# facebookresearch/detectron2

Hardware: NVIDIA H100
Metric: Mask R-CNN R50-FPN training hot-path images/sec (custom-op path fwd+bwd, 2 images/GPU) (higher is better)
Workload: dtype f32

## Files before the change

detectron2_b200/_C.py:

```python
import ctypes as C
import os

import torch

_HERE = os.path.dirname(os.path.abspath(__file__))
LIB_PATH = os.path.join(_HERE, "libd2b200.so")

_lib = None

D2B_ERRORS = {-1: "invalid argument", -2: "workspace too small", -3: "unsupported configuration"}


class DcnParams(C.Structure):
    _fields_ = [(n, C.c_int) for n in ("N", "Cin", "H", "W", "Cout", "kh", "kw", "stride_h", "stride_w", "pad_h",
                                        "pad_w", "dil_h", "dil_w", "groups", "deformable_groups")]


MAX_LEVELS = 8
MAX_IMAGES = 64
ABI_VERSION = 4
DCN_X_NHWC = 1
ROI_ROTATED, ROI_BACKWARD = 1, 2
DTYPE_CODE = {torch.float32: 0, torch.float16: 1, torch.bfloat16: 2}
MATCH_ROTATED, MATCH_LOW_QUALITY, MATCH_APPEND_GT = 1, 2, 4
MATCH_MAX_THRESHOLDS = 8


class Pyramid(C.Structure):
    _fields_ = [("num_levels", C.c_int), ("feat", C.c_void_p * MAX_LEVELS), ("grad", C.c_void_p * MAX_LEVELS),
                ("H", C.c_int * MAX_LEVELS), ("W", C.c_int * MAX_LEVELS), ("scale", C.c_float * MAX_LEVELS),
                ("min_level", C.c_int), ("max_level", C.c_int), ("canonical_level", C.c_int),
                ("canonical_box_size", C.c_float), ("level_rois", C.c_void_p)]


class RpnLevels(C.Structure):
    _fields_ = [("num_levels", C.c_int), ("proposals", C.c_void_p * MAX_LEVELS), ("topk_idx", C.c_void_p * MAX_LEVELS),
                ("topk_scores", C.c_void_p * MAX_LEVELS), ("A", C.c_int * MAX_LEVELS), ("k", C.c_int * MAX_LEVELS)]


class DenseLevels(C.Structure):
    _fields_ = [("num_levels", C.c_int), ("anchors", C.c_void_p * MAX_LEVELS), ("deltas", C.c_void_p * MAX_LEVELS),
                ("topk_idx", C.c_void_p * MAX_LEVELS), ("topk_scores", C.c_void_p * MAX_LEVELS),
                ("R", C.c_int * MAX_LEVELS), ("k", C.c_int * MAX_LEVELS)]


LABELS_I8, LABELS_I64 = 0, 1
SAMPLE_MAX_SAMPLES = 8192
LOSS_STATUS_INVALID_BOX, LOSS_STATUS_INVALID_CLASS, LOSS_STATUS_INVALID_BOX_ORDER = 1, 2, 4
LOSS_TYPES = {"smooth_l1": 0, "giou": 1}


class DenseLossLevels(C.Structure):
    _fields_ = [("num_levels", C.c_int), ("logits", C.c_void_p * MAX_LEVELS), ("deltas", C.c_void_p * MAX_LEVELS),
                ("grad_logits", C.c_void_p * MAX_LEVELS), ("grad_deltas", C.c_void_p * MAX_LEVELS),
                ("R", C.c_int * MAX_LEVELS)]


def _declare(lib):
    vp, f32p, i64p, u8p = C.c_void_p, C.c_void_p, C.c_void_p, C.c_void_p
    i, f, d, sz, i64 = C.c_int, C.c_float, C.c_double, C.c_size_t, C.c_int64
    sig = {
        "d2b_abi_version": (i, []),
        "d2b_cuda_version": (i, []),
        "d2b_arch": (C.c_char_p, []),
        "d2b_roi_align_forward": (i, [f32p, i, i, i, i, f32p, i, f, i, i, i, i, f32p, vp]),
        "d2b_roi_align_backward": (i, [f32p, f32p, i, f, i, i, i, i, i, i, i, i, f32p, vp]),
        "d2b_roi_pooler_forward": (i, [C.POINTER(Pyramid), i, i, f32p, i, i, i, i, i, f32p, vp]),
        "d2b_roi_pooler_backward": (i, [C.POINTER(Pyramid), i, i, f32p, f32p, i, i, i, i, i, vp]),
        "d2b_roi_align_forward_nhwc": (i, [f32p, i, i, i, i, f32p, i, f, i, i, i, i, f32p, vp]),
        "d2b_roi_pooler_forward_nhwc": (i, [C.POINTER(Pyramid), i, i, f32p, i, i, i, i, i, f32p, vp]),
        "d2b_pyramid_nchw_to_nhwc": (i, [C.POINTER(Pyramid), i, i, C.POINTER(C.c_void_p), vp]),
        "d2b_pyramid_nhwc_to_nchw": (i, [C.POINTER(Pyramid), i, i, C.POINTER(C.c_void_p), vp]),
        "d2b_pyramid_nchw_to_nhwc_t": (i, [C.POINTER(Pyramid), i, i, C.POINTER(C.c_void_p), i, vp]),
        "d2b_pyramid_nhwc_to_nchw_t": (i, [C.POINTER(Pyramid), i, i, C.POINTER(C.c_void_p), i, vp]),
        "d2b_roi_pooler_forward_nhwc_t": (i, [C.POINTER(Pyramid), i, i, f32p, i, i, i, i, i, vp, i, vp]),
        "d2b_roi_pooler_backward_nhwc_t": (i, [C.POINTER(Pyramid), i, i, vp, i, f32p, i, i, i, i, i, vp]),
        "d2b_roi_align_backward_nhwc": (i, [f32p, f32p, i, f, i, i, i, i, i, i, i, i, f32p, vp]),
        "d2b_roi_pooler_backward_nhwc": (i, [C.POINTER(Pyramid), i, i, f32p, f32p, i, i, i, i, i, vp]),
        "d2b_roi_align_rotated_forward": (i, [f32p, i, i, i, i, f32p, i, f, i, i, i, f32p, vp]),
        "d2b_roi_align_rotated_backward": (i, [f32p, f32p, i, f, i, i, i, i, i, i, i, f32p, vp]),
        "d2b_roi_align_rotated_forward_nhwc": (i, [f32p, i, i, i, i, f32p, i, f, i, i, i, f32p, vp]),
        "d2b_roi_align_rotated_backward_nhwc": (i, [f32p, f32p, i, f, i, i, i, i, i, i, i, f32p, vp]),
        "d2b_roi_pooler_rotated_forward": (i, [C.POINTER(Pyramid), i, i, f32p, i, i, i, i, f32p, vp]),
        "d2b_roi_pooler_rotated_backward": (i, [C.POINTER(Pyramid), i, i, f32p, f32p, i, i, i, i, vp]),
        "d2b_roi_pooler_rotated_forward_nhwc_t": (i, [C.POINTER(Pyramid), i, i, f32p, i, i, i, i, vp, i, vp]),
        "d2b_roi_pooler_rotated_backward_nhwc_t": (i, [C.POINTER(Pyramid), i, i, vp, i, f32p, i, i, i, i, vp]),
        "d2b_roi_pooler_nhwc_supported": (i, [C.POINTER(Pyramid), i, i, i, i]),
        "d2b_nms_workspace_bytes": (sz, [i64, i, i64]),
        "d2b_nms": (i, [f32p, f32p, i64p, i64, d, i, i64, i64p, i64p, vp, sz, vp]),
        "d2b_rpn_prepare": (i, [C.POINTER(RpnLevels), i, f32p, f, i, f32p, f32p, f32p, f32p, i64p, vp, vp]),
        "d2b_rpn_select": (i, [i64p, i64p, i, i, i, f32p, f32p, i64p, f32p, f32p, i64p, i64p, vp]),
        "d2b_frcnn_prepare": (i, [f32p, f32p, C.POINTER(C.c_int), i, i, i, f32p, f, i, f32p, f32p, f32p, f32p, i64p, i64p,
                                  i64p, i64p, vp]),
        "d2b_dense_prepare": (i, [C.POINTER(DenseLevels), i, i, C.POINTER(C.c_float), f, f32p, f32p, f32p, f32p, i64p, i64p,
                                  vp]),
        "d2b_rrpn_prepare": (i, [C.POINTER(RpnLevels), i, f32p, f, i, f32p, f32p, f32p, f32p, i64p, vp, vp]),
        "d2b_frcnn_rotated_prepare": (i, [f32p, f32p, C.POINTER(C.c_int), i, i, i, f32p, f, i, i, f32p, f32p, f32p, f32p, i64p,
                                          i64p, i64p, i64p, vp]),
        "d2b_rpn_select_rotated": (i, [i64p, i64p, i, i, i, f32p, f32p, i64p, f32p, f32p, i64p, i64p, vp]),
        "d2b_mask_loss_forward": (i, [f32p, i, i, i, u8p, i, i, i, f32p, i64p, i64p, f32p, u8p, vp]),
        "d2b_mask_loss_backward": (i, [f32p, i, i, i, u8p, i64p, f32p, f32p, vp]),
        "d2b_keypoints_workspace_bytes": (sz, [i, i]),
        "d2b_keypoints_from_heatmaps": (i, [f32p, i, i, i, f32p, f32p, vp, sz, vp]),
        "d2b_keypoint_loss_forward": (i, [vp, i, i, i, i, f32p, f32p, i64p, u8p, f32p, i64p, vp]),
        "d2b_keypoint_loss_backward": (i, [vp, i, i, i, i, i64p, u8p, f32p, vp, vp]),
        "d2b_dense_loss_workspace_bytes": (sz, [C.POINTER(DenseLossLevels), i, i, i]),
        "d2b_dense_loss_forward": (i, [C.POINTER(DenseLossLevels), i, i, i, i, f32p, f32p, vp, i, f, f, f, i, f,
                                       C.POINTER(C.c_float), f32p, f32p, i64p, i64p, vp, vp, sz, vp]),
        "d2b_dense_loss_backward": (i, [C.POINTER(DenseLossLevels), i, i, i, i, f32p, f32p, vp, i, f, f, f, i, f,
                                        C.POINTER(C.c_float), f32p, f32p, vp]),
        "d2b_frcnn_loss_workspace_bytes": (sz, [i]),
        "d2b_frcnn_loss_forward": (i, [vp, vp, i, i, i, i, i, f32p, f32p, i64p, f, i, f, C.POINTER(C.c_float), f32p, f32p, i64p,
                                       i64p, i64p, i64p, vp, vp, sz, vp]),
        "d2b_frcnn_loss_backward": (i, [vp, vp, i, i, i, i, i, f32p, f32p, i64p, f, i, f, C.POINTER(C.c_float), f32p, f32p, vp,
                                        vp, vp]),
        "d2b_box_iou_rotated": (i, [f32p, i64, f32p, i64, f32p, vp]),
        "d2b_match_workspace_bytes": (sz, [i, i, i]),
        "d2b_match_boxes": (i, [f32p, i64p, i, i, f32p, i64, i64p, i, C.POINTER(C.c_double), i, C.POINTER(C.c_int), i, f32p, d,
                                i64p, i64, i64p, vp, f32p, i64p, vp, vp, sz, vp]),
        "d2b_sample_labels_workspace_bytes": (sz, [i, i, i]),
        "d2b_sample_labels": (i, [vp, i, i, i, i64, i, i, vp, vp, i64p, i64p, i64p, vp, sz, vp]),
        "d2b_deform_conv_tc_shape_supported": (i, [C.POINTER(DcnParams), i]),
        "d2b_deform_conv_forward_workspace_bytes": (sz, [C.POINTER(DcnParams), i, i]),
        "d2b_deform_conv_cols_bytes": (sz, [C.POINTER(DcnParams), i]),
        "d2b_deform_conv_forward": (i, [f32p, f32p, f32p, f32p, f32p, C.POINTER(DcnParams), i, i, f32p, vp, vp, sz, vp]),
        "d2b_deform_conv_backward_workspace_bytes": (sz, [C.POINTER(DcnParams), i, i, i, i]),
        "d2b_deform_conv_backward": (i, [f32p, f32p, f32p, f32p, f32p, C.POINTER(DcnParams), i, i, vp, f32p, f32p, f32p,
                                         f32p, f32p, vp, sz, vp]),
        "d2b_deform_conv_fused_forward": (i, [f32p, f32p, f32p, f32p, f32p, i, C.POINTER(DcnParams), i, i, f32p, vp, vp, sz,
                                              vp]),
        "d2b_deform_conv_fused_backward": (i, [f32p, f32p, f32p, f32p, i, f32p, f32p, C.POINTER(DcnParams), i, i, vp, f32p,
                                               f32p, f32p, vp, sz, vp]),
        "d2b_paste_masks": (i, [f32p, f32p, i, i, i, i, f, u8p, vp]),
        "d2b_paste_masks_packed": (i, [f32p, f32p, i, i, i, i, f, vp, vp]),
    }
    for name, (res, args) in sig.items():
        fn = getattr(lib, name)
        fn.restype = res
        fn.argtypes = args
    return sig


EXPORTED = None


def lib():
    global _lib, EXPORTED
    if _lib is None:
        if not os.path.exists(LIB_PATH):
            raise RuntimeError(
                "detectron2_b200: native library %s is missing. Build it with `python -m detectron2_b200.build` "
                "(or __graft_entry__.build()). There is no CPU / PyTorch fallback for these ops." % LIB_PATH)
        l = C.CDLL(LIB_PATH)
        EXPORTED = _declare(l)
        if l.d2b_abi_version() != ABI_VERSION:
            raise RuntimeError("libd2b200.so ABI version mismatch")
        _lib = l
    return _lib


def check(rc, what):
    if rc == 0:
        return
    if rc < 0:
        raise RuntimeError("%s: %s (d2b error %d)" % (what, D2B_ERRORS.get(rc, "error"), rc))
    raise RuntimeError("%s: CUDA error %d" % (what, rc))


def stream_ptr(device):
    return C.c_void_p(torch.cuda.current_stream(device).cuda_stream)


def ptr(t):
    return None if t is None else C.c_void_p(t.data_ptr())


def require_cuda(*tensors):
    for t in tensors:
        if t is not None and not t.is_cuda:
            raise NotImplementedError("detectron2_b200 ops run on CUDA tensors only (no CPU fallback)")


def get_cuda_version():
    v = lib().d2b_cuda_version()
    return "CUDA %d.%d" % (v // 1000, (v % 1000) // 10)


def has_cuda():
    return True


def get_compiler_version():
    return "nvcc (sm_90a)"


DCN_PRECISION = -1


def _into(dst, src):
    if dst.shape != src.shape:
        dst.resize_(src.shape)
    dst.copy_(src)


def deform_conv_forward(input, weight, offset, output, columns, ones, kW, kH, dW, dH, padW, padH, dilW, dilH, group,
                        deformable_group, im2col_step):
    from . import ops

    if weight.shape[3] != kW or weight.shape[2] != kH:
        raise RuntimeError("deform_conv_forward: kernel size does not match the weight tensor")
    y = ops.deform_conv_op(input, offset, None, weight, None, [dH, dW], [padH, padW], [dilH, dilW], group, deformable_group,
                           DCN_PRECISION)
    _into(output, y)
    return 1


def deform_conv_backward_input(input, offset, gradOutput, gradInput, gradOffset, weight, columns, kW, kH, dW, dH, padW,
                               padH, dilW, dilH, group, deformable_group, im2col_step):
    from . import ops

    gx, go, _, _, _ = ops.deform_conv_backward_op(input, offset, None, weight, gradOutput, [dH, dW], [padH, padW],
                                                  [dilH, dilW], group, deformable_group, False, True, False, DCN_PRECISION)
    _into(gradInput, gx)
    _into(gradOffset, go)
    return 1


def deform_conv_backward_filter(input, offset, gradOutput, gradWeight, columns, ones, kW, kH, dW, dH, padW, padH, dilW,
                                dilH, group, deformable_group, scale, im2col_step):
    from . import ops

    _, _, _, gw, _ = ops.deform_conv_backward_op(input, offset, None, gradWeight.new_empty(gradWeight.shape), gradOutput,
                                                 [dH, dW], [padH, padW], [dilH, dilW], group, deformable_group, False,
                                                 False, True, DCN_PRECISION)
    gradWeight.add_(gw, alpha=float(scale))
    return 1


def modulated_deform_conv_forward(input, weight, bias, ones, offset, mask, output, columns, kernel_h, kernel_w, stride_h,
                                  stride_w, pad_h, pad_w, dilation_h, dilation_w, group, deformable_group, with_bias):
    from . import ops

    y = ops.deform_conv_op(input, offset, mask, weight, bias if with_bias else None, [stride_h, stride_w], [pad_h, pad_w],
                           [dilation_h, dilation_w], group, deformable_group, DCN_PRECISION)
    _into(output, y)


def modulated_deform_conv_backward(input, weight, bias, ones, offset, mask, columns, grad_input, grad_weight, grad_bias,
                                   grad_offset, grad_mask, grad_output, kernel_h, kernel_w, stride_h, stride_w, pad_h,
                                   pad_w, dilation_h, dilation_w, group, deformable_group, with_bias):
    from . import ops

    gx, go, gm, gw, gb = ops.deform_conv_backward_op(input, offset, mask, weight, grad_output, [stride_h, stride_w],
                                                     [pad_h, pad_w], [dilation_h, dilation_w], group, deformable_group,
                                                     bool(with_bias), True, True, DCN_PRECISION)
    _into(grad_input, gx)
    _into(grad_offset, go)
    _into(grad_mask, gm)
    grad_weight.add_(gw)
    if with_bias:
        grad_bias.add_(gb)
```

detectron2_b200/csrc/deform_conv.cu:

```cuda
#include "common.cuh"
#include "deform_conv_tc.cuh"

namespace {

constexpr int BN = 64;
constexpr int BM = 64;
constexpr int BK = 16;
constexpr int kThreads = 256;

struct Dims {
  int N, Cin, H, W, Cout, kh, kw, sh, sw, ph, pw, dh, dw, G, DG, Ho, Wo;
  int cpg, opg, cpdg, KK, HoWo;
};

inline bool make_dims(const d2b_dcn_params* p, Dims& d) {
  if (!p) return false;
  d.N = p->N; d.Cin = p->Cin; d.H = p->H; d.W = p->W; d.Cout = p->Cout; d.kh = p->kh; d.kw = p->kw;
  d.sh = p->stride_h; d.sw = p->stride_w; d.ph = p->pad_h; d.pw = p->pad_w; d.dh = p->dil_h; d.dw = p->dil_w;
  d.G = p->groups; d.DG = p->deformable_groups;
  if (d.N < 0 || d.Cin <= 0 || d.H <= 0 || d.W <= 0 || d.Cout <= 0 || d.kh <= 0 || d.kw <= 0 || d.sh <= 0 ||
      d.sw <= 0 || d.ph < 0 || d.pw < 0 || d.dh <= 0 || d.dw <= 0 || d.G <= 0 || d.DG <= 0)
    return false;
  if (d.Cin % d.G || d.Cout % d.G || d.Cin % d.DG) return false;
  d.Ho = (d.H + 2 * d.ph - (d.dh * (d.kh - 1) + 1)) / d.sh + 1;
  d.Wo = (d.W + 2 * d.pw - (d.dw * (d.kw - 1) + 1)) / d.sw + 1;
  if (d.Ho <= 0 || d.Wo <= 0) return false;
  d.cpg = d.Cin / d.G; d.opg = d.Cout / d.G; d.cpdg = d.Cin / d.DG; d.KK = d.kh * d.kw; d.HoWo = d.Ho * d.Wo;
  return true;
}

struct TapTile {
  int pos[4][BN];
  float wgt[4][BN];
  float msk[BN];
  float fh[BN], fw[BN];
  int inside[BN];
};

__device__ __forceinline__ void build_taps(TapTile& t, const Dims& d, const float* __restrict__ offset,
                                           const float* __restrict__ mask, int b, int dg, int kp, int p0) {
  for (int n = threadIdx.x; n < BN; n += kThreads) {
    const int p = p0 + n;
    int pos[4] = {-1, -1, -1, -1};
    float w[4] = {0.f, 0.f, 0.f, 0.f};
    float m = 1.f, lh = 0.f, lw = 0.f;
    int inside = 0;
    if (p < d.HoWo) {
      const int ho = p / d.Wo, wo = p - ho * d.Wo;
      const int i = kp / d.kw, j = kp - i * d.kw;
      const size_t obase = ((size_t)(b * d.DG + dg) * 2 * d.KK) * d.HoWo;
      const float oh = offset[obase + (size_t)(2 * kp) * d.HoWo + p];
      const float ow = offset[obase + (size_t)(2 * kp + 1) * d.HoWo + p];
      const float h = (float)(ho * d.sh - d.ph + i * d.dh) + oh;
      const float wv = (float)(wo * d.sw - d.pw + j * d.dw) + ow;
      if (mask) m = mask[((size_t)(b * d.DG + dg) * d.KK + kp) * d.HoWo + p];
      if (h > -1.f && wv > -1.f && h < (float)d.H && wv < (float)d.W) {
        inside = 1;
        const int hl = (int)floorf(h), wl = (int)floorf(wv);
        lh = h - (float)hl;
        lw = wv - (float)wl;
        const float hh = 1.f - lh, hw = 1.f - lw;
        const bool t0 = hl >= 0, t1 = hl + 1 <= d.H - 1, l0 = wl >= 0, l1 = wl + 1 <= d.W - 1;
        if (t0 && l0) { pos[0] = hl * d.W + wl; w[0] = hh * hw; }
        if (t0 && l1) { pos[1] = hl * d.W + wl + 1; w[1] = hh * lw; }
        if (t1 && l0) { pos[2] = (hl + 1) * d.W + wl; w[2] = lh * hw; }
        if (t1 && l1) { pos[3] = (hl + 1) * d.W + wl + 1; w[3] = lh * lw; }
      }
    }
#pragma unroll
    for (int q = 0; q < 4; ++q) {
      t.pos[q][n] = pos[q];
      t.wgt[q][n] = w[q];
    }
    t.msk[n] = m;
    t.fh[n] = lh;
    t.fw[n] = lw;
    t.inside[n] = inside;
  }
}

__device__ __forceinline__ float gather_val(const TapTile& t, const float* __restrict__ plane, int n) {
  float v = 0.f;
#pragma unroll
  for (int q = 0; q < 4; ++q) {
    const int pos = t.pos[q][n];
    if (pos >= 0) v += t.wgt[q][n] * __ldg(plane + pos);
  }
  return v;
}

__global__ void __launch_bounds__(kThreads) dcn_fwd_kernel(const float* __restrict__ x,
                                                           const float* __restrict__ offset,
                                                           const float* __restrict__ mask,
                                                           const float* __restrict__ weight,
                                                           const float* __restrict__ bias, Dims d,
                                                           float* __restrict__ out) {
  __shared__ TapTile taps;
  __shared__ float As[BK][BM + 4];
  __shared__ float Bs[BK][BN + 4];
  const int p0 = blockIdx.x * BN, m0 = blockIdx.y * BM;
  const int b = blockIdx.z / d.G, g = blockIdx.z - b * d.G;
  const int tid = threadIdx.x, tx = tid & 15, ty = tid >> 4;
  const int K = d.cpg * d.KK;
  float acc[4][4] = {};
  const int cbeg = g * d.cpg, cend = cbeg + d.cpg;
  for (int dg = cbeg / d.cpdg; dg * d.cpdg < cend; ++dg) {
    const int sbeg = max(cbeg, dg * d.cpdg), send = min(cend, (dg + 1) * d.cpdg);
    for (int kp = 0; kp < d.KK; ++kp) {
      __syncthreads();
      build_taps(taps, d, offset, mask, b, dg, kp, p0);
      __syncthreads();
      for (int c0 = sbeg; c0 < send; c0 += BK) {
        for (int e = tid; e < BK * BM; e += kThreads) {
          const int kk = e / BM, m = e - kk * BM;
          const int c = c0 + kk;
          float v = 0.f;
          if (c < send && m0 + m < d.opg) v = __ldg(weight + (size_t)(g * d.opg + m0 + m) * K + (c - cbeg) * d.KK + kp);
          As[kk][m] = v;
        }
        for (int e = tid; e < BK * BN; e += kThreads) {
          const int kk = e / BN, n = e - kk * BN;
          const int c = c0 + kk;
          float v = 0.f;
          if (c < send) v = gather_val(taps, x + ((size_t)b * d.Cin + c) * d.H * d.W, n) * taps.msk[n];
          Bs[kk][n] = v;
        }
        __syncthreads();
#pragma unroll
        for (int kk = 0; kk < BK; ++kk) {
          float a[4], bb[4];
#pragma unroll
          for (int i = 0; i < 4; ++i) a[i] = As[kk][ty * 4 + i];
#pragma unroll
          for (int j = 0; j < 4; ++j) bb[j] = Bs[kk][tx * 4 + j];
#pragma unroll
          for (int i = 0; i < 4; ++i)
#pragma unroll
            for (int j = 0; j < 4; ++j) acc[i][j] = fmaf(a[i], bb[j], acc[i][j]);
        }
        __syncthreads();
      }
    }
  }
#pragma unroll
  for (int i = 0; i < 4; ++i) {
    const int m = m0 + ty * 4 + i;
    if (m >= d.opg) continue;
    const int oc = g * d.opg + m;
    const float bv = bias ? bias[oc] : 0.f;
#pragma unroll
    for (int j = 0; j < 4; ++j) {
      const int p = p0 + tx * 4 + j;
      if (p < d.HoWo) out[((size_t)b * d.Cout + oc) * d.HoWo + p] = acc[i][j] + bv;
    }
  }
}

__global__ void __launch_bounds__(kThreads) dcn_bwd_data_kernel(const float* __restrict__ x,
                                                                const float* __restrict__ offset,
                                                                const float* __restrict__ mask,
                                                                const float* __restrict__ weight,
                                                                const float* __restrict__ gout, Dims d,
                                                                float* __restrict__ gx, float* __restrict__ goff,
                                                                float* __restrict__ gmask) {
  __shared__ TapTile taps;
  __shared__ float Ws[BK][BK + 1];
  __shared__ float Gs[BK][BN + 4];
  __shared__ float red[3][4][BN];
  const int p0 = blockIdx.x * BN;
  const int b = blockIdx.z / d.G, g = blockIdx.z - b * d.G;
  const int tid = threadIdx.x, n = tid & 63, kq = tid >> 6;
  const int K = d.cpg * d.KK;
  const int cbeg = g * d.cpg, cend = cbeg + d.cpg;
  const size_t plane = (size_t)d.H * d.W;
  for (int dg = cbeg / d.cpdg; dg * d.cpdg < cend; ++dg) {
    const int sbeg = max(cbeg, dg * d.cpdg), send = min(cend, (dg + 1) * d.cpdg);
    for (int kp = 0; kp < d.KK; ++kp) {
      __syncthreads();
      build_taps(taps, d, offset, mask, b, dg, kp, p0);
      __syncthreads();
      float s_h = 0.f, s_w = 0.f, s_m = 0.f;
      for (int c0 = sbeg + (int)blockIdx.y * BK; c0 < send; c0 += BK * (int)gridDim.y) {
        float acc[4] = {0.f, 0.f, 0.f, 0.f};
        for (int mm0 = 0; mm0 < d.opg; mm0 += BK) {
          {
            const int m = tid >> 4, kk = tid & 15;
            const int c = c0 + kk;
            float v = 0.f;
            if (c < send && mm0 + m < d.opg)
              v = __ldg(weight + (size_t)(g * d.opg + mm0 + m) * K + (c - cbeg) * d.KK + kp);
            Ws[m][kk] = v;
          }
          for (int e = tid; e < BK * BN; e += kThreads) {
            const int m = e / BN, nn = e - m * BN;
            float v = 0.f;
            if (mm0 + m < d.opg && p0 + nn < d.HoWo)
              v = __ldg(gout + ((size_t)b * d.Cout + g * d.opg + mm0 + m) * d.HoWo + p0 + nn);
            Gs[m][nn] = v;
          }
          __syncthreads();
#pragma unroll
          for (int m = 0; m < BK; ++m) {
            const float gv = Gs[m][n];
#pragma unroll
            for (int i = 0; i < 4; ++i) acc[i] = fmaf(Ws[m][kq + 4 * i], gv, acc[i]);
          }
          __syncthreads();
        }
        if (taps.inside[n]) {
          const float mk = taps.msk[n], lh = taps.fh[n], lw = taps.fw[n];
          const int q0 = taps.pos[0][n], q1 = taps.pos[1][n], q2 = taps.pos[2][n], q3 = taps.pos[3][n];
#pragma unroll
          for (int i = 0; i < 4; ++i) {
            const int c = c0 + kq + 4 * i;
            if (c >= send) continue;
            const float gc = acc[i];
            const float gm = gc * mk;
            const float* __restrict__ xp = x + ((size_t)b * d.Cin + c) * plane;
            float* __restrict__ gp = gx ? gx + ((size_t)b * d.Cin + c) * plane : nullptr;
            const float v0 = q0 >= 0 ? __ldg(xp + q0) : 0.f, v1 = q1 >= 0 ? __ldg(xp + q1) : 0.f;
            const float v2 = q2 >= 0 ? __ldg(xp + q2) : 0.f, v3 = q3 >= 0 ? __ldg(xp + q3) : 0.f;
            if (gp) {
              if (q0 >= 0) atomicAdd(gp + q0, gm * taps.wgt[0][n]);
              if (q1 >= 0) atomicAdd(gp + q1, gm * taps.wgt[1][n]);
              if (q2 >= 0) atomicAdd(gp + q2, gm * taps.wgt[2][n]);
              if (q3 >= 0) atomicAdd(gp + q3, gm * taps.wgt[3][n]);
            }
            s_h += gm * ((1.f - lw) * (v2 - v0) + lw * (v3 - v1));
            s_w += gm * ((1.f - lh) * (v1 - v0) + lh * (v3 - v2));
            s_m += gc * (taps.wgt[0][n] * v0 + taps.wgt[1][n] * v1 + taps.wgt[2][n] * v2 + taps.wgt[3][n] * v3);
          }
        }
      }
      red[0][kq][n] = s_h;
      red[1][kq][n] = s_w;
      red[2][kq][n] = s_m;
      __syncthreads();
      if (tid < 3 * BN) {
        const int which = tid / BN, nn = tid - which * BN;
        const int p = p0 + nn;
        if (p < d.HoWo) {
          const float v = red[which][0][nn] + red[which][1][nn] + red[which][2][nn] + red[which][3][nn];
          if (which < 2) {
            if (goff) atomicAdd(goff + ((size_t)(b * d.DG + dg) * 2 * d.KK + 2 * kp + which) * d.HoWo + p, v);
          } else if (gmask && mask) {
            atomicAdd(gmask + ((size_t)(b * d.DG + dg) * d.KK + kp) * d.HoWo + p, v);
          }
        }
      }
    }
  }
}

__global__ void __launch_bounds__(kThreads) dcn_bwd_weight_kernel(const float* __restrict__ x,
                                                                  const float* __restrict__ offset,
                                                                  const float* __restrict__ mask,
                                                                  const float* __restrict__ gout, Dims d,
                                                                  int tiles_per_cta, int n_ctile,
                                                                  float* __restrict__ gw) {
  __shared__ TapTile taps;
  __shared__ float Gs[BN][BM + 4];
  __shared__ float Cs[BN][BK + 1];
  const int g = blockIdx.z;
  const int mt = blockIdx.y / n_ctile, ct = blockIdx.y - mt * n_ctile;
  const int m0 = mt * BM;
  const int cbeg = g * d.cpg;
  const int c0 = cbeg + ct * BK;
  const int cend = min(cbeg + d.cpg, c0 + BK);
  const int tid = threadIdx.x, tm = tid >> 2, tc = tid & 3;
  const int K = d.cpg * d.KK;
  const int ptiles = d2b_cdiv(d.HoWo, BN);
  const int total_tiles = d.N * ptiles;
  const int t_begin = blockIdx.x * tiles_per_cta, t_end = min(total_tiles, t_begin + tiles_per_cta);
  for (int kp = 0; kp < d.KK; ++kp) {
    float acc[4] = {0.f, 0.f, 0.f, 0.f};
    for (int t = t_begin; t < t_end; ++t) {
      const int b = t / ptiles, p0 = (t - b * ptiles) * BN;
      for (int cs = c0; cs < cend;) {
        const int dg = cs / d.cpdg;
        const int ce = min(cend, (dg + 1) * d.cpdg);
        __syncthreads();
        build_taps(taps, d, offset, mask, b, dg, kp, p0);
        for (int e = tid; e < BN * BM; e += kThreads) {
          const int nn = e & 63, m = e >> 6;
          float v = 0.f;
          if (m0 + m < d.opg && p0 + nn < d.HoWo)
            v = __ldg(gout + ((size_t)b * d.Cout + g * d.opg + m0 + m) * d.HoWo + p0 + nn);
          Gs[nn][m] = v;
        }
        __syncthreads();
        for (int e = tid; e < BN * BK; e += kThreads) {
          const int nn = e & 63, kk = e >> 6;
          const int c = c0 + kk;
          float v = 0.f;
          if (c >= cs && c < ce) v = gather_val(taps, x + ((size_t)b * d.Cin + c) * d.H * d.W, nn) * taps.msk[nn];
          Cs[nn][kk] = v;
        }
        __syncthreads();
#pragma unroll 8
        for (int nn = 0; nn < BN; ++nn) {
          const float gv = Gs[nn][tm];
#pragma unroll
          for (int i = 0; i < 4; ++i) acc[i] = fmaf(gv, Cs[nn][tc * 4 + i], acc[i]);
        }
        cs = ce;
      }
    }
    if (m0 + tm < d.opg) {
#pragma unroll
      for (int i = 0; i < 4; ++i) {
        const int c = c0 + tc * 4 + i;
        if (c < cend) atomicAdd(gw + (size_t)(g * d.opg + m0 + tm) * K + (c - cbeg) * d.KK + kp, acc[i]);
      }
    }
  }
}

__global__ void __launch_bounds__(256) dcn_bias_grad_kernel(const float* __restrict__ gout, int N, int Cout, int HoWo,
                                                            float* __restrict__ gb) {
  __shared__ float s[8];
  const int oc = blockIdx.x;
  float v = 0.f;
  for (int b = 0; b < N; ++b)
    for (int p = threadIdx.x; p < HoWo; p += 256) v += gout[((size_t)b * Cout + oc) * HoWo + p];
  for (int o = 16; o; o >>= 1) v += __shfl_xor_sync(0xffffffffu, v, o);
  if ((threadIdx.x & 31) == 0) s[threadIdx.x >> 5] = v;
  __syncthreads();
  if (threadIdx.x == 0) {
    float t = 0.f;
    for (int i = 0; i < 8; ++i) t += s[i];
    gb[oc] = t;
  }
}

}

D2B_API int d2b_deform_conv_tc_shape_supported(const d2b_dcn_params* p, int backward) {
  return backward ? d2b_deform_conv_tc_bwd_supported(p) : d2b_deform_conv_tc_supported(p);
}

D2B_API size_t d2b_deform_conv_forward_workspace_bytes(const d2b_dcn_params* p, int precision, int flags) {
  if (precision == 0) return 0;
  if (precision == -1 && !d2b_deform_conv_tc_supported(p)) return 0;
  return d2b_deform_conv_tc_fwd_workspace(p, (flags & D2B_DCN_X_NHWC) ? 1 : 0);
}

D2B_API size_t d2b_deform_conv_cols_bytes(const d2b_dcn_params* p, int precision) {
  if (precision == -1) precision = (d2b_deform_conv_tc_supported(p) && d2b_deform_conv_tc_bwd_supported(p)) ? 1 : 0;
  if (precision == 0 || !d2b_deform_conv_tc_bwd_supported(p)) return 0;
  return d2b_deform_conv_tc_cols_bytes(p, precision);
}

D2B_API int d2b_deform_conv_forward(const float* x, const float* offset, const float* mask, const float* weight,
                                    const float* bias, const d2b_dcn_params* p, int precision, int flags, float* out,
                                    void* cols, void* workspace, size_t workspace_bytes, void* stream) {
  Dims d;
  if (!make_dims(p, d)) return D2B_EINVAL;
  if (d.N == 0) return D2B_OK;
  if (!x || !offset || !weight || !out) return D2B_EINVAL;
  if (precision < -1 || precision > 2) return D2B_EINVAL;
  if (precision == -1) precision = d2b_deform_conv_tc_supported(p) ? 1 : 0;
  if (precision != 0)
    return d2b_deform_conv_forward_tc(x, offset, mask, weight, nullptr, bias, 0, p, precision,
                                      (flags & D2B_DCN_X_NHWC) ? 1 : 0, out, cols, workspace, workspace_bytes, stream);
  if (flags & D2B_DCN_X_NHWC) return D2B_EUNSUPPORTED;
  if (cols) return D2B_EINVAL;
  dim3 grid(d2b_cdiv(d.HoWo, BN), d2b_cdiv(d.opg, BM), d.N * d.G);
  dcn_fwd_kernel<<<grid, kThreads, 0, (cudaStream_t)stream>>>(x, offset, mask, weight, bias, d, out);
  D2B_CHECK_LAUNCH();
  return D2B_OK;
}

D2B_API size_t d2b_deform_conv_backward_workspace_bytes(const d2b_dcn_params* p, int precision, int flags, int need_data,
                                                        int need_weight) {
  if (precision == 0) return 0;
  if (precision == -1 && !d2b_deform_conv_tc_bwd_supported(p)) return 0;
  return d2b_deform_conv_tc_bwd_workspace(p, (flags & D2B_DCN_X_NHWC) ? 1 : 0, need_data, need_weight);
}

D2B_API int d2b_deform_conv_backward(const float* x, const float* offset, const float* mask, const float* weight,
                                     const float* grad_out, const d2b_dcn_params* p, int precision, int flags,
                                     const void* cols, float* grad_x, float* grad_offset, float* grad_mask,
                                     float* grad_weight, float* grad_bias, void* workspace, size_t workspace_bytes,
                                     void* stream_) {
  cudaStream_t stream = (cudaStream_t)stream_;
  Dims d;
  if (!make_dims(p, d)) return D2B_EINVAL;
  if (precision < -1 || precision > 2) return D2B_EINVAL;
  if (precision == -1) precision = d2b_deform_conv_tc_bwd_supported(p) ? 1 : 0;
  if (d.N > 0 && (!x || !offset || !weight || !grad_out)) return D2B_EINVAL;
  if (cols && precision == 0) return D2B_EINVAL;
  if (grad_bias) {
    if (d.N == 0) {
      D2B_CUDA(cudaMemsetAsync(grad_bias, 0, (size_t)d.Cout * 4, stream));
    } else {
      dcn_bias_grad_kernel<<<d.Cout, 256, 0, stream>>>(grad_out, d.N, d.Cout, d.HoWo, grad_bias);
      D2B_CHECK_LAUNCH();
    }
  }
  if (precision != 0)
    return d2b_deform_conv_backward_tc(x, offset, mask, weight, grad_out, nullptr, nullptr, 0, p, precision,
                                       (flags & D2B_DCN_X_NHWC) ? 1 : 0, cols, grad_x, grad_offset, grad_mask, grad_weight,
                                       workspace, workspace_bytes, stream_);
  if (flags & D2B_DCN_X_NHWC) return D2B_EUNSUPPORTED;
  const size_t nx = (size_t)d.N * d.Cin * d.H * d.W, noff = (size_t)d.N * d.DG * 2 * d.KK * d.HoWo;
  const size_t nm = (size_t)d.N * d.DG * d.KK * d.HoWo, nw = (size_t)d.Cout * d.cpg * d.KK;
  if (grad_x && nx) D2B_CUDA(cudaMemsetAsync(grad_x, 0, nx * 4, stream));
  if (grad_offset && noff) D2B_CUDA(cudaMemsetAsync(grad_offset, 0, noff * 4, stream));
  if (grad_mask && nm) D2B_CUDA(cudaMemsetAsync(grad_mask, 0, nm * 4, stream));
  if (grad_weight) D2B_CUDA(cudaMemsetAsync(grad_weight, 0, nw * 4, stream));
  if (d.N == 0) return D2B_OK;
  if (grad_x || grad_offset || grad_mask) {
    const int base_ctas = d2b_cdiv(d.HoWo, BN) * d.N * d.G;
    int csplit = d2b_cdiv(3LL * d2b_num_sms(), base_ctas);
    const int nchunks = d2b_cdiv(d.cpg, BK);
    if (csplit > nchunks) csplit = nchunks;
    if (csplit < 1) csplit = 1;
    dim3 grid(d2b_cdiv(d.HoWo, BN), csplit, d.N * d.G);
    dcn_bwd_data_kernel<<<grid, kThreads, 0, stream>>>(x, offset, mask, weight, grad_out, d, grad_x, grad_offset,
                                                       grad_mask);
    D2B_CHECK_LAUNCH();
  }
  if (grad_weight) {
    const int ptiles = d2b_cdiv(d.HoWo, BN), total = d.N * ptiles;
    const int n_ctile = d2b_cdiv(d.cpg, BK), n_mtile = d2b_cdiv(d.opg, BM);
    int per_tile_ctas = n_ctile * n_mtile * d.G;
    int splits = d2b_cdiv(4LL * d2b_num_sms(), per_tile_ctas);
    if (splits > total) splits = total;
    if (splits < 1) splits = 1;
    const int tiles_per_cta = d2b_cdiv(total, splits);
    splits = d2b_cdiv(total, tiles_per_cta);
    dim3 grid(splits, n_mtile * n_ctile, d.G);
    dcn_bwd_weight_kernel<<<grid, kThreads, 0, stream>>>(x, offset, mask, grad_out, d, tiles_per_cta, n_ctile,
                                                         grad_weight);
    D2B_CHECK_LAUNCH();
  }
  return D2B_OK;
}

D2B_API int d2b_deform_conv_fused_forward(const float* x, const float* offset_mask, const float* weight, const float* scale,
                                          const float* shift, int relu, const d2b_dcn_params* p, int precision, int flags,
                                          float* out, void* cols, void* workspace, size_t workspace_bytes, void* stream) {
  Dims d;
  if (!make_dims(p, d)) return D2B_EINVAL;
  if (d.N == 0) return D2B_OK;
  if (!x || !offset_mask || !weight || !out || precision == 0 || precision < -1 || precision > 2) return D2B_EINVAL;
  if (precision == -1) precision = 1;
  return d2b_deform_conv_forward_tc(x, offset_mask, nullptr, weight, scale, shift, relu, p, precision,
                                    ((flags & D2B_DCN_X_NHWC) ? 1 : 0) | 2, out, cols, workspace, workspace_bytes, stream);
}

D2B_API int d2b_deform_conv_fused_backward(const float* x, const float* offset_mask, const float* weight, const float* scale,
                                           int relu, const float* y, const float* grad_out, const d2b_dcn_params* p,
                                           int precision, int flags, const void* cols, float* grad_x,
                                           float* grad_offset_mask, float* grad_weight, void* workspace,
                                           size_t workspace_bytes, void* stream) {
  Dims d;
  if (!make_dims(p, d)) return D2B_EINVAL;
  if (precision == 0 || precision < -1 || precision > 2) return D2B_EINVAL;
  if (precision == -1) precision = 1;
  if (d.N > 0 && (!x || !offset_mask || !weight || !grad_out)) return D2B_EINVAL;
  return d2b_deform_conv_backward_tc(x, offset_mask, nullptr, weight, grad_out, scale, y, relu, p, precision,
                                     ((flags & D2B_DCN_X_NHWC) ? 1 : 0) | 2, cols, grad_x, grad_offset_mask, nullptr,
                                     grad_weight, workspace, workspace_bytes, stream);
}
```

detectron2_b200/csrc/deform_conv_tc.cu:

```cuda
#include <algorithm>
#include <cstdlib>

#include "common.cuh"
#include "deform_conv_tc.cuh"
#include "tc_common.cuh"

using namespace d2b_tc;

namespace {

constexpr int kWorkerWarps = 16;
constexpr int kWorkers = kWorkerWarps * 32;
constexpr int kThreads = kWorkers + 128;
constexpr int kLaunchRegs = (65536 / kThreads) & ~7;
constexpr int kWorkerRegs = 112, kSideRegs = 24;
static_assert(kWorkers * kWorkerRegs + (kThreads - kWorkers) * kSideRegs <= kThreads * kLaunchRegs,
              "register budget exceeds the launch allocation");
constexpr int kMaxBN = 128;
constexpr int kRowsPerHalf = 128 / (2 * kWorkerWarps);
constexpr int kTile = 16384;
constexpr int kMaxSmem = 227 * 1024;
constexpr int kGcolPitch = 132;

struct TC {
  int N, Cin, H, W, Cout, kh, kw, sh, sw, ph, pw, dh, dw, G, DG, Ho, Wo, cpg, opg, cpdg, KK, HoWo;
  int pack, SG, cps, ops, cbs, U;
  int tiles_img;
  int stages_img;
  int MC;
  int nks;
  long long off_bs, mask_bs;
  int mask_sigmoid;
};

struct Epi {
  const float* scale;
  const float* shift;
  int relu;
};

struct K1P { int BN, noct, goct, nkp, ksplit, S, tap_bytes, stage_bytes, red; };
struct K2P { int mper, msplit, tap_bytes; };
struct K3P { int BN, noct, sper, nsplit, S, stage_bytes; };

inline size_t align256(size_t v) { return (v + 255) & ~(size_t)255; }

bool make_tc(const d2b_dcn_params* p, TC& d) {
  if (!p) return false;
  d.N = p->N; d.Cin = p->Cin; d.H = p->H; d.W = p->W; d.Cout = p->Cout; d.kh = p->kh; d.kw = p->kw;
  d.sh = p->stride_h; d.sw = p->stride_w; d.ph = p->pad_h; d.pw = p->pad_w; d.dh = p->dil_h; d.dw = p->dil_w;
  d.G = p->groups; d.DG = p->deformable_groups;
  if (d.N < 0 || d.Cin <= 0 || d.H <= 0 || d.W <= 0 || d.Cout <= 0 || d.kh <= 0 || d.kw <= 0 || d.sh <= 0 || d.sw <= 0 ||
      d.ph < 0 || d.pw < 0 || d.dh <= 0 || d.dw <= 0 || d.G <= 0 || d.DG <= 0)
    return false;
  if (d.Cin % d.G || d.Cout % d.G || d.Cin % d.DG) return false;
  d.Ho = (d.H + 2 * d.ph - (d.dh * (d.kh - 1) + 1)) / d.sh + 1;
  d.Wo = (d.W + 2 * d.pw - (d.dw * (d.kw - 1) + 1)) / d.sw + 1;
  if (d.Ho <= 0 || d.Wo <= 0) return false;
  d.cpg = d.Cin / d.G; d.opg = d.Cout / d.G; d.cpdg = d.Cin / d.DG; d.KK = d.kh * d.kw; d.HoWo = d.Ho * d.Wo;
  if (d.cpg >= 64) {
    if (d.cpg % 64) return false;
    d.pack = 1;
  } else {
    if (d.cpg != 16 && d.cpg != 32) return false;
    d.pack = 64 / d.cpg;
    if (d.G % d.pack) return false;
  }
  if (d.cpdg % 64) return false;
  d.SG = d.G / d.pack; d.cps = d.cpg * d.pack; d.ops = d.opg * d.pack; d.cbs = d.cps / 64; d.U = d.KK * d.cbs;
  if (d.ops % 16) return false;
  if (d.KK > 49) return false;
  if ((long long)d.H * d.W * d.Cin >= (1LL << 29)) return false;
  if ((long long)d.HoWo * d.Cout >= (1LL << 31) || (long long)d.Cout * d.cpg * d.KK >= (1LL << 31)) return false;
  d.tiles_img = d2b_cdiv(d.HoWo, 128);
  d.stages_img = d2b_cdiv(d.HoWo, 64);
  d.MC = (d.U + 1) / 2;
  d.nks = d.ops / 64;
  if ((long long)d.N * d.tiles_img > 0x7fffffffLL) return false;
  d.off_bs = (long long)d.DG * 2 * d.KK * d.HoWo;
  d.mask_bs = (long long)d.DG * d.KK * d.HoWo;
  d.mask_sigmoid = 0;
  return true;
}

const float* use_fused_offset_mask(TC& d, const float* offset_mask) {
  d.off_bs = d.mask_bs = (long long)d.DG * 3 * d.KK * d.HoWo;
  d.mask_sigmoid = 1;
  return offset_mask + (size_t)d.DG * 2 * d.KK * d.HoWo;
}

int largest_tile(int n) {
  for (int t = kMaxBN; t >= 16; t >>= 1)
    if (n % t == 0) return t;
  return 0;
}

int best_split(long long base, int work, int max_split, int overhead) {
  int best = 1;
  long long best_cost = -1;
  for (int s = 1; s <= max_split; ++s) {
    const int per = d2b_cdiv(work, s);
    const int parts = d2b_cdiv(work, per);
    const long long cost = (long long)d2b_cdiv(base * parts, d2b_num_sms()) * (per + overhead);
    if (best_cost < 0 || cost < best_cost) {
      best_cost = cost;
      best = parts;
    }
  }
  return best;
}

bool plan_k1(const TC& d, K1P& k, bool colfed = false) {
  k.BN = largest_tile(d.ops);
  if (k.BN < 16) return false;
  k.noct = d.ops / k.BN;
  k.goct = colfed ? 1 : k.noct;
  const int base = d.N * d.tiles_img * d.SG * k.goct;
  k.ksplit = best_split(base, d.KK, d.KK, 1);
  k.nkp = d2b_cdiv(d.KK, k.ksplit);
  k.ksplit = d2b_cdiv(d.KK, k.nkp);
  k.red = k.ksplit > 1;
  const int ndg = d.DG == 1 ? 1 : std::min(d.DG, d2b_cdiv(d.cps, d.cpdg) + 1);
  k.tap_bytes = ndg * k.nkp * 128 * 16;
  k.stage_bytes = 2 * kTile + 2 * k.BN * 128;
  k.S = 3;
  while (k.S > 1 && k.S * k.stage_bytes + k.tap_bytes + 1024 + 128 > kMaxSmem) --k.S;
  return k.S >= 2;
}

bool plan_k1c(const TC& d, K1P& k1, K1P& kc) {
  const long long base = (long long)d.N * d.tiles_img * d.SG * (k1.noct - 1);
  if (k1.goct != 1 || k1.noct < 2 || (long long)d.N * d.tiles_img * (k1.noct - 1) > 0x7fffffffLL) return false;
  kc = k1;
  kc.goct = k1.noct - 1;
  kc.ksplit = best_split(base, d.KK, d.KK, 1);
  kc.nkp = d2b_cdiv(d.KK, kc.ksplit);
  kc.ksplit = d2b_cdiv(d.KK, kc.nkp);
  kc.tap_bytes = 0;
  kc.S = 3;
  while (kc.S > 1 && kc.S * kc.stage_bytes + 1024 + 128 > kMaxSmem) --kc.S;
  if (kc.S < 2) return false;
  k1.red = kc.red = k1.ksplit > 1 || kc.ksplit > 1;
  return true;
}

bool plan_k2(const TC& d, K2P& k) {
  if (d.ops % 64) return false;
  const int base = d.N * d.tiles_img * d.SG;
  k.msplit = best_split(base, d.MC, d.MC, 1);
  k.mper = d2b_cdiv(d.MC, k.msplit);
  k.msplit = d2b_cdiv(d.MC, k.mper);
  const int nkp = std::min(d.KK, (2 * k.mper + d.cbs - 1) / d.cbs + 1);
  const int ndg = d.DG == 1 ? 1 : std::min(d.DG, d2b_cdiv(d.cps, d.cpdg) + 1);
  k.tap_bytes = ndg * nkp * 128 * 16;
  return 2 * 4 * kTile + 128 * kGcolPitch * 4 + k.tap_bytes + 1024 + 128 <= kMaxSmem;
}

bool plan_k3(const TC& d, K3P& k) {
  if (d.ops % 64) return false;
  k.BN = largest_tile(d.ops);
  k.noct = d.ops / k.BN;
  const int units = d.MC * d.SG * k.noct;
  const int total = d.N * d.stages_img;
  k.nsplit = best_split(units, total, std::min(total, 4 * d2b_num_sms()), 3);
  k.sper = d2b_cdiv(total, k.nsplit);
  k.nsplit = d2b_cdiv(total, k.sper);
  k.stage_bytes = 2 * kTile + 2 * k.BN * 128;
  k.S = 3;
  while (k.S > 1 && k.S * k.stage_bytes + 4096 + 1024 + 128 > kMaxSmem) --k.S;
  return k.S >= 2;
}

struct TapRaw {
  float oh, ow, m;
};

__device__ __forceinline__ TapRaw tap_loads(const TC& d, const float* __restrict__ offset, const float* __restrict__ mask,
                                            int b, int dg, int kp, int p) {
  TapRaw r = {0.f, 0.f, 1.f};
  if (p < d.HoWo) {
    const size_t ob = (size_t)b * d.off_bs + ((size_t)dg * 2 * d.KK) * d.HoWo;
    r.oh = __ldg(offset + ob + (size_t)(2 * kp) * d.HoWo + p);
    r.ow = __ldg(offset + ob + (size_t)(2 * kp + 1) * d.HoWo + p);
    if (mask) r.m = __ldg(mask + (size_t)b * d.mask_bs + ((size_t)dg * d.KK + kp) * d.HoWo + p);
  }
  return r;
}

__device__ __forceinline__ int4 tap_finish(const TC& d, const TapRaw& r, bool has_mask, int kp, int p) {
  int4 t = make_int4(0, 0, 0, 0);
  if (p < d.HoWo) {
    const int ho = p / d.Wo, wo = p - ho * d.Wo;
    const int ki = kp / d.kw, kj = kp - ki * d.kw;
    const float hf = (float)(ho * d.sh - d.ph + ki * d.dh) + r.oh;
    const float wf = (float)(wo * d.sw - d.pw + kj * d.dw) + r.ow;
    float m = r.m;
    if (has_mask && d.mask_sigmoid) m = 1.f / (1.f + expf(-m));
    if (hf > -1.f && wf > -1.f && hf < (float)d.H && wf < (float)d.W) {
      const float hfl = floorf(hf), wfl = floorf(wf);
      const int hl = (int)hfl, wl = (int)wfl;
      const bool t0 = hl >= 0, t1 = hl + 1 <= d.H - 1, l0 = wl >= 0, l1 = wl + 1 <= d.W - 1;
      const int flags = (t0 && l0 ? 1 : 0) | (t0 && l1 ? 2 : 0) | (t1 && l0 ? 4 : 0) | (t1 && l1 ? 8 : 0);
      t.x = ((hl * d.W + wl + d.W + 1) << 4) | flags;
      t.y = __float_as_int(hf - hfl);
      t.z = __float_as_int(wf - wfl);
      t.w = __float_as_int(m);
    }
  }
  return t;
}

__device__ __forceinline__ int4 make_tap(const TC& d, const float* __restrict__ offset, const float* __restrict__ mask,
                                         int b, int dg, int kp, int p) {
  return tap_finish(d, tap_loads(d, offset, mask, b, dg, kp, p), mask != nullptr, kp, p);
}

struct Taps4 {
  float4 v0, v1, v2, v3;
};

__device__ __forceinline__ void load_corners(const float* __restrict__ xcb, uint32_t Cin, uint32_t rs, int code, Taps4& t) {
  const float* __restrict__ p = xcb + (uint32_t)(code >> 4) * Cin;
  const float4 z = make_float4(0.f, 0.f, 0.f, 0.f);
  t.v0 = (code & 1) ? __ldg(reinterpret_cast<const float4*>(p)) : z;
  t.v1 = (code & 2) ? __ldg(reinterpret_cast<const float4*>(p + Cin)) : z;
  t.v2 = (code & 4) ? __ldg(reinterpret_cast<const float4*>(p + rs)) : z;
  t.v3 = (code & 8) ? __ldg(reinterpret_cast<const float4*>(p + (rs + Cin))) : z;
}

__device__ __forceinline__ void interp4(const Taps4& t, float w0, float w1, float w2, float w3, float (&v)[4]) {
  const F2 z = f2_pack(0.f, 0.f), p0 = f2_pack(w0, w0), p1 = f2_pack(w1, w1), p2 = f2_pack(w2, w2), p3 = f2_pack(w3, w3);
  F2 a = f2_fma(p0, f2_pack(t.v0.x, t.v0.y), z), b = f2_fma(p0, f2_pack(t.v0.z, t.v0.w), z);
  a = f2_fma(p1, f2_pack(t.v1.x, t.v1.y), a);
  b = f2_fma(p1, f2_pack(t.v1.z, t.v1.w), b);
  a = f2_fma(p2, f2_pack(t.v2.x, t.v2.y), a);
  b = f2_fma(p2, f2_pack(t.v2.z, t.v2.w), b);
  a = f2_fma(p3, f2_pack(t.v3.x, t.v3.y), a);
  b = f2_fma(p3, f2_pack(t.v3.z, t.v3.w), b);
  f2_unpack(a, v[0], v[1]);
  f2_unpack(b, v[2], v[3]);
}

__device__ __forceinline__ void gather_store(const Taps4& t, int4 tap, uint8_t* a_hi, uint8_t* a_lo, uint32_t off,
                                             bool split) {
  const float lh = __int_as_float(tap.y), lw = __int_as_float(tap.z), m = __int_as_float(tap.w);
  const float hh = 1.f - lh, hw = 1.f - lw;
  float v[4];
  interp4(t, hh * hw * m, hh * lw * m, lh * hw * m, lh * lw * m, v);
  uint2 hi, lo;
  split4(v, hi, lo);
  *reinterpret_cast<uint2*>(a_hi + off) = hi;
  if (split) *reinterpret_cast<uint2*>(a_lo + off) = lo;
}

template <int BN, int kTransA, int kSplit>
__device__ __forceinline__ void mma_stage_(float (&acc)[BN / 4], uint32_t a_hi, uint32_t a_lo, uint32_t b_hi, uint32_t b_lo) {
  const int g = (threadIdx.x >> 7);
  const uint32_t ao = kTransA ? (uint32_t)(g & 1) * 8192u : (uint32_t)(g & 1) * 64u * 128u;
  const uint32_t bo = (uint32_t)(g >> 1) * (uint32_t)(BN / 2) * 128u;
  const uint32_t lbo = kTransA ? 8192u : 0u;
  wgmma_fence();
#pragma unroll
  for (int kk = 0; kk < 4; ++kk) {
    const uint32_t ak = ao + (kTransA ? (uint32_t)kk * 2048u : (uint32_t)kk * 32u), bk = bo + (uint32_t)kk * 32u;
    Wgmma<BN / 2, kTransA>::mma(acc, wgmma_desc(a_hi + ak, lbo, 1024), wgmma_desc(b_hi + bk, 0, 1024), 1);
    if (kSplit) {
      Wgmma<BN / 2, kTransA>::mma(acc, wgmma_desc(a_hi + ak, lbo, 1024), wgmma_desc(b_lo + bk, 0, 1024), 1);
      Wgmma<BN / 2, kTransA>::mma(acc, wgmma_desc(a_lo + ak, lbo, 1024), wgmma_desc(b_hi + bk, 0, 1024), 1);
    }
  }
  wgmma_commit();
}
template <int BN, int kTransA>
__device__ __forceinline__ void mma_stage(float (&acc)[BN / 4], uint32_t a_hi, uint32_t a_lo, uint32_t b_hi, uint32_t b_lo,
                                          int split) {
  if (split) mma_stage_<BN, kTransA, 1>(acc, a_hi, a_lo, b_hi, b_lo);
  else mma_stage_<BN, kTransA, 0>(acc, a_hi, a_lo, b_hi, b_lo);
}

template <int BN>
__device__ __forceinline__ int acc_row(int i) {
  const int t = threadIdx.x & 127;
  return (threadIdx.x >> 7 & 1) * 64 + (t >> 5) * 16 + ((t & 31) >> 2) + ((i >> 1) & 1) * 8;
}
template <int BN>
__device__ __forceinline__ int acc_col(int i) {
  return (threadIdx.x >> 8) * (BN / 2) + (i >> 2) * 8 + (threadIdx.x & 3) * 2 + (i & 1);
}

template <int BN>
__device__ __forceinline__ void fwd_epilogue(const float (&acc)[BN / 4], const Epi& ep, const TC& d, const K1P& k,
                                             float* __restrict__ out, int b, int p0, int oc0) {
  const bool add_shift = ep.shift != nullptr && blockIdx.z == 0;
#pragma unroll
  for (int i = 0; i < BN / 4; ++i) {
    const int p = p0 + acc_row<BN>(i);
    if (p >= d.HoWo) continue;
    const int oc = oc0 + acc_col<BN>(i);
    float* dst = out + ((size_t)b * d.Cout + oc) * d.HoWo + p;
    float v = acc[i];
    if (k.red) {
      red_add(dst, v + ((add_shift && !ep.scale && !ep.relu) ? __ldg(ep.shift + oc) : 0.f));
    } else {
      if (ep.scale) v *= __ldg(ep.scale + oc);
      if (ep.shift) v += __ldg(ep.shift + oc);
      if (ep.relu) v = fmaxf(v, 0.f);
      *dst = v;
    }
  }
}

template <int BN>
__global__ void __launch_bounds__(kThreads, 1) dcn_fwd_tc_kernel(const float* __restrict__ xh,
                                                                   const float* __restrict__ offset,
                                                                   const float* __restrict__ mask,
                                                                   const uint8_t* __restrict__ wt, const Epi ep, const TC d,
                                                                   const K1P k, const int split, float* __restrict__ out,
                                                                   uint8_t* __restrict__ cols) {
  extern __shared__ uint8_t smem_raw[];
  uint8_t* smem = smem_raw + ((1024u - (smem_u32(smem_raw) & 1023u)) & 1023u);
  int4* taps = reinterpret_cast<int4*>(smem + k.S * k.stage_bytes);
  uint64_t* bars = reinterpret_cast<uint64_t*>(reinterpret_cast<uint8_t*>(taps) + k.tap_bytes);
  uint64_t* full_bar = bars;
  uint64_t* empty_bar = bars + k.S;

  const int tid = threadIdx.x, warp = tid >> 5, lane = tid & 31;
  const int b = blockIdx.x / d.tiles_img, p0 = (blockIdx.x - b * d.tiles_img) * 128;
  const int sg = blockIdx.y / k.goct, oct = blockIdx.y - sg * k.goct;
  const int kp0 = blockIdx.z * k.nkp, nkp = min(d.KK, kp0 + k.nkp) - kp0;
  const int nt = nkp * d.cbs;
  const int dg0 = (sg * d.cps) / d.cpdg;
  const bool saving = cols != nullptr && oct == 0;

  if (tid == 0) {
    for (int s = 0; s < k.S; ++s) {
      mbar_init(&full_bar[s], kWorkerWarps + 1);
      mbar_init(&empty_bar[s], kWorkerWarps + (saving ? 1 : 0));
    }
    mbar_init_fence();
  }
  if (tid < kWorkers) {
    const int ndg = ((sg + 1) * d.cps - 1) / d.cpdg - dg0 + 1;
    for (int i = tid; i < ndg * nkp * 128; i += kWorkers) {
      const int row = i & 127, r = i >> 7;
      const int dgl = r / nkp, kpl = r - dgl * nkp;
      taps[i] = make_tap(d, offset, mask, b, dg0 + dgl, kp0 + kpl, p0 + row);
    }
  }
  __syncthreads();
  if (warp < kWorkerWarps) reg_alloc<kWorkerRegs>();
  else reg_dealloc<kSideRegs>();

  if (warp < kWorkerWarps) {
    const int half = lane >> 4, q = lane & 15;
    const float* __restrict__ ximg = xh + (size_t)b * d.H * d.W * d.Cin - (size_t)(d.W + 1) * d.Cin;
    const uint32_t ucin = (uint32_t)d.Cin, urs = (uint32_t)(d.W * d.Cin);
    float acc[BN / 4];
#pragma unroll
    for (int i = 0; i < BN / 4; ++i) acc[i] = 0.f;
    int kpl = 0, cb = 0;
    auto stage = [&](int t) {
      const int s = t % k.S;
      const uint32_t par = (uint32_t)((t / k.S) & 1);
      const int cbase = sg * d.cps + cb * 64;
      const int4* __restrict__ tp = taps + ((cbase / d.cpdg - dg0) * nkp + kpl) * 128;
      const float* __restrict__ xc = ximg + cbase + q * 4;
      uint8_t* a_hi = smem + s * k.stage_bytes;
      uint8_t* a_lo = a_hi + kTile;
      mbar_wait(&empty_bar[s], par ^ 1u);
      {
        int4 tap[kRowsPerHalf];
        Taps4 c[kRowsPerHalf];
#pragma unroll
        for (int j = 0; j < kRowsPerHalf; ++j) tap[j] = tp[warp * 2 * kRowsPerHalf + j * 2 + half];
#pragma unroll
        for (int j = 0; j < kRowsPerHalf; ++j) load_corners(xc, ucin, urs, tap[j].x, c[j]);
#pragma unroll
        for (int j = 0; j < kRowsPerHalf; ++j) {
          const uint32_t r = (uint32_t)(warp * 2 * kRowsPerHalf + j * 2 + half);
          gather_store(c[j], tap[j], a_hi, a_lo, swz128(r, (uint32_t)(q >> 1)) + (uint32_t)(q & 1) * 8u, split != 0);
        }
      }
      fence_proxy_async();
      __syncwarp();
      if (lane == 0) mbar_arrive(&full_bar[s]);
      mbar_wait(&full_bar[s], par);
      const uint32_t sa = smem_u32(a_hi), sb = sa + 2 * kTile;
      mma_stage<BN, 0>(acc, sa, sa + kTile, sb, sb + (uint32_t)BN * 128u, split);
      if (++cb == d.cbs) { cb = 0; ++kpl; }
    };
    stage(0);
    for (int t = 1; t < nt; ++t) {
      stage(t);
      wgmma_wait<1>();
      __syncwarp();
      if (lane == 0) mbar_arrive(&empty_bar[(t - 1) % k.S]);
    }
    wgmma_wait<0>();
    fwd_epilogue<BN>(acc, ep, d, k, out, b, p0, sg * d.ops + oct * k.BN);
  } else if (warp == kWorkerWarps) {
    if (lane == 0) {
      const uint32_t bytes = (uint32_t)(split ? 2 : 1) * (uint32_t)k.BN * 128u;
      for (int t = 0; t < nt; ++t) {
        const int s = t % k.S;
        const uint32_t par = (uint32_t)((t / k.S) & 1);
        mbar_wait(&empty_bar[s], par ^ 1u);
        const size_t tile = ((size_t)(sg * k.noct + oct) * d.U + (size_t)kp0 * d.cbs + t);
        mbar_arrive_expect_tx(&full_bar[s], bytes);
        bulk_g2s(smem + s * k.stage_bytes + 2 * kTile, wt + tile * (size_t)(2 * k.BN * 128), bytes, &full_bar[s]);
      }
    }
  } else if (warp == kWorkerWarps + 1) {
    if (saving && lane == 0) {
      const uint32_t tile_bytes = (uint32_t)(split ? 2 : 1) * (uint32_t)kTile;
      for (int t = 0; t < nt; ++t) {
        const int s = t % k.S;
        const uint32_t par = (uint32_t)((t / k.S) & 1);
        mbar_wait(&full_bar[s], par);
        const size_t tile = ((size_t)blockIdx.x * d.SG + sg) * d.U + (size_t)kp0 * d.cbs + t;
        bulk_s2g(cols + tile * tile_bytes, smem + s * k.stage_bytes, tile_bytes);
        bulk_commit();
        bulk_wait_read0();
        mbar_arrive(&empty_bar[s]);
      }
      bulk_wait0();
    }
  }
}

template <int BN>
__global__ void __launch_bounds__(kThreads, 1) dcn_fwd_cols_kernel(const uint8_t* __restrict__ cols,
                                                                   const uint8_t* __restrict__ wt, const Epi ep, const TC d,
                                                                   const K1P k, const int split, float* __restrict__ out) {
  extern __shared__ uint8_t smem_raw[];
  uint8_t* smem = smem_raw + ((1024u - (smem_u32(smem_raw) & 1023u)) & 1023u);
  uint64_t* bars = reinterpret_cast<uint64_t*>(smem + k.S * k.stage_bytes);
  uint64_t* full_bar = bars;
  uint64_t* empty_bar = bars + k.S;

  const int tid = threadIdx.x, warp = tid >> 5, lane = tid & 31;
  const int tile = blockIdx.x / k.goct, oct = 1 + (blockIdx.x - tile * k.goct);
  const int b = tile / d.tiles_img, p0 = (tile - b * d.tiles_img) * 128;
  const int sg = blockIdx.y;
  const int kp0 = blockIdx.z * k.nkp, nkp = min(d.KK, kp0 + k.nkp) - kp0;
  const int nt = nkp * d.cbs;

  if (tid == 0) {
    for (int s = 0; s < k.S; ++s) {
      mbar_init(&full_bar[s], 1);
      mbar_init(&empty_bar[s], kWorkerWarps);
    }
    mbar_init_fence();
  }
  __syncthreads();
  if (warp < kWorkerWarps) reg_alloc<kWorkerRegs>();
  else reg_dealloc<kSideRegs>();

  if (warp < kWorkerWarps) {
    float acc[BN / 4];
#pragma unroll
    for (int i = 0; i < BN / 4; ++i) acc[i] = 0.f;
    auto issue = [&](int t) {
      const int s = t % k.S;
      mbar_wait(&full_bar[s], (uint32_t)((t / k.S) & 1));
      const uint32_t sa = smem_u32(smem + s * k.stage_bytes), sb = sa + 2 * kTile;
      mma_stage<BN, 0>(acc, sa, sa + kTile, sb, sb + (uint32_t)BN * 128u, split);
    };
    issue(0);
    for (int t = 1; t < nt; ++t) {
      issue(t);
      wgmma_wait<1>();
      __syncwarp();
      if (lane == 0) mbar_arrive(&empty_bar[(t - 1) % k.S]);
    }
    wgmma_wait<0>();
    fwd_epilogue<BN>(acc, ep, d, k, out, b, p0, sg * d.ops + oct * k.BN);
  } else if (warp == kWorkerWarps) {
    if (lane == 0) {
      const uint32_t parts = split ? 2u : 1u;
      const uint32_t abytes = parts * (uint32_t)kTile;
      const size_t u0 = (size_t)kp0 * d.cbs;
      const uint8_t* asrc = cols + (((size_t)tile * d.SG + sg) * d.U + u0) * abytes;
      const uint8_t* bsrc = wt + ((size_t)(sg * k.noct + oct) * d.U + u0) * (size_t)(2 * BN * 128);
      int s = 0;
      uint32_t par = 1u;
      for (int t = nt; t > 0; --t, asrc += abytes, bsrc += 2 * BN * 128) {
        mbar_wait(&empty_bar[s], par);
        mbar_arrive_expect_tx(&full_bar[s], abytes / 128u * (128u + BN));
        bulk_g2s(smem + s * k.stage_bytes, asrc, abytes, &full_bar[s]);
        bulk_g2s(smem + s * k.stage_bytes + 2 * kTile, bsrc, abytes / 128u * BN, &full_bar[s]);
        if (++s == k.S) {
          s = 0;
          par ^= 1u;
        }
      }
    }
  }
}

__global__ void __launch_bounds__(kThreads, 1) dcn_bwd_data_tc_kernel(const float* __restrict__ xh,
                                                                      const float* __restrict__ offset,
                                                                      const float* __restrict__ mask,
                                                                      const uint8_t* __restrict__ gt,
                                                                      const uint8_t* __restrict__ wt, const TC d,
                                                                      const K2P k, const int split,
                                                                      float* __restrict__ gxh, float* __restrict__ goff,
                                                                      float* __restrict__ gmask) {
  extern __shared__ uint8_t smem_raw[];
  uint8_t* smem = smem_raw + ((1024u - (smem_u32(smem_raw) & 1023u)) & 1023u);
  constexpr int kStage = 4 * kTile;
  float* gcol = reinterpret_cast<float*>(smem + 2 * kStage);
  int4* taps = reinterpret_cast<int4*>(smem + 2 * kStage + 128 * kGcolPitch * 4);
  uint64_t* bars = reinterpret_cast<uint64_t*>(reinterpret_cast<uint8_t*>(taps) + k.tap_bytes);
  uint64_t* full_bar = bars;
  uint64_t* empty_bar = bars + 2;

  const int tid = threadIdx.x, warp = tid >> 5, lane = tid & 31;
  const int b = blockIdx.x / d.tiles_img, pt = blockIdx.x - b * d.tiles_img, p0 = pt * 128;
  const int sg = blockIdx.y;
  const int m0 = blockIdx.z * k.mper, m1 = min(d.MC, m0 + k.mper), nm = m1 - m0;
  const int u_begin = 2 * m0, u_end = min(d.U, 2 * m1);
  const int kp0 = u_begin / d.cbs, nkp = (u_end - 1) / d.cbs - kp0 + 1;
  const int dg0 = (sg * d.cps) / d.cpdg;

  if (tid == 0) {
    for (int s = 0; s < 2; ++s) {
      mbar_init(&full_bar[s], 1);
      mbar_init(&empty_bar[s], kWorkerWarps);
    }
    mbar_init_fence();
  }
  if (tid < kWorkers) {
    const int ndg = ((sg + 1) * d.cps - 1) / d.cpdg - dg0 + 1;
    for (int i = tid; i < ndg * nkp * 128; i += kWorkers) {
      const int row = i & 127, r = i >> 7;
      const int dgl = r / nkp, kpl = r - dgl * nkp;
      taps[i] = make_tap(d, offset, mask, b, dg0 + dgl, kp0 + kpl, p0 + row);
    }
  }
  __syncthreads();
  if (warp < kWorkerWarps) reg_alloc<kWorkerRegs>();
  else reg_dealloc<kSideRegs>();

  if (warp < kWorkerWarps) {
    const int half = lane >> 4, q = lane & 15;
    const size_t img_off = (size_t)b * d.H * d.W * d.Cin - (size_t)(d.W + 1) * d.Cin;
    const float* __restrict__ ximg = xh + img_off;
    float* __restrict__ gimg = gxh ? gxh + img_off : nullptr;
    const uint32_t ucin = (uint32_t)d.Cin, urs = (uint32_t)(d.W * d.Cin);
    constexpr int R = kRowsPerHalf;
    float sh[R], sw[R], sm[R];
#pragma unroll
    for (int j = 0; j < R; ++j) sh[j] = sw[j] = sm[j] = 0.f;
    int cur_kp = -1, cur_dg = -1;

    auto flush = [&]() {
      if (cur_kp < 0) return;
      static_assert(R == 4, "the reduction below is written for 4 rows per half-warp");
      float v12[12];
#pragma unroll
      for (int j = 0; j < R; ++j) {
        v12[3 * j] = sh[j];
        v12[3 * j + 1] = sw[j];
        v12[3 * j + 2] = sm[j];
      }
      const bool b8 = q & 8, b4 = q & 4, b2 = q & 2, b1 = q & 1;
      float v6[6], v3[3];
#pragma unroll
      for (int i = 0; i < 6; ++i) {
        const float keep = b8 ? v12[i + 6] : v12[i], send = b8 ? v12[i] : v12[i + 6];
        v6[i] = keep + __shfl_xor_sync(0xffffffffu, send, 8);
      }
#pragma unroll
      for (int i = 0; i < 3; ++i) {
        const float keep = b4 ? v6[i + 3] : v6[i], send = b4 ? v6[i] : v6[i + 3];
        v3[i] = keep + __shfl_xor_sync(0xffffffffu, send, 4);
      }
      const float k0 = b2 ? v3[2] : v3[0], s0 = b2 ? v3[0] : v3[2];
      const float k1 = b2 ? 0.f : v3[1], s1 = b2 ? v3[1] : 0.f;
      const float u0 = k0 + __shfl_xor_sync(0xffffffffu, s0, 2);
      const float u1 = k1 + __shfl_xor_sync(0xffffffffu, s1, 2);
      float v = (b1 ? u1 : u0) + __shfl_xor_sync(0xffffffffu, b1 ? u0 : u1, 1);
      {
        const int j = q >> 2, which = q & 3;
        const int row = warp * 2 * R + j * 2 + half;
        const int p = p0 + row;
        if (which < 3 && p < d.HoWo) {
          if (which < 2) {
            if (goff) red_add(goff + (size_t)b * d.off_bs + ((size_t)cur_dg * 2 * d.KK + 2 * cur_kp + which) * d.HoWo + p, v);
          } else if (gmask) {
            if (d.mask_sigmoid) {
              const float m = __int_as_float(taps[((cur_dg - dg0) * nkp + (cur_kp - kp0)) * 128 + row].w);
              v *= m * (1.f - m);
            }
            red_add(gmask + (size_t)b * d.mask_bs + ((size_t)cur_dg * d.KK + cur_kp) * d.HoWo + p, v);
          }
        }
      }
#pragma unroll
      for (int j = 0; j < R; ++j) sh[j] = sw[j] = sm[j] = 0.f;
    };

    for (int ml = 0; ml < nm; ++ml) {
      const int buf = ml & 1;
      const int m = m0 + ml;
      const int nu = (2 * m + 1 < d.U) ? 2 : 1;
      {
        float acc[32];
#pragma unroll
        for (int i = 0; i < 32; ++i) acc[i] = 0.f;
        for (int ks = 0; ks < d.nks; ++ks) {
          const int c = ml * d.nks + ks, s = c & 1;
          mbar_wait(&full_bar[s], (uint32_t)((c >> 1) & 1));
          const uint32_t sa = smem_u32(smem + s * kStage);
          mma_stage<128, 0>(acc, sa, sa + kTile, sa + 2 * kTile, sa + 3 * kTile, split);
          wgmma_wait<0>();
          __syncwarp();
          if (lane == 0) mbar_arrive(&empty_bar[s]);
        }
#pragma unroll
        for (int i = 0; i < 32; i += 2)
          *reinterpret_cast<float2*>(gcol + acc_row<128>(i) * kGcolPitch + acc_col<128>(i)) = make_float2(acc[i], acc[i + 1]);
      }
      named_bar_sync(1, kWorkers);
      for (int ul = 0; ul < nu; ++ul) {
        const int u = 2 * m + ul;
        const int kp = u / d.cbs, cb = u - kp * d.cbs;
        const int cbase = sg * d.cps + cb * 64;
        const int dg = cbase / d.cpdg;
        if (kp != cur_kp || dg != cur_dg) {
          flush();
          cur_kp = kp;
          cur_dg = dg;
        }
        const int4* __restrict__ tp = taps + ((dg - dg0) * nkp + (kp - kp0)) * 128;
        const float* __restrict__ xc = ximg + cbase + q * 4;
        float* __restrict__ gc = gimg + cbase + q * 4;
        constexpr int kB2 = 2;
#pragma unroll
        for (int it = 0; it < R / kB2; ++it) {
          int4 tap[kB2];
          Taps4 c[kB2];
#pragma unroll
          for (int e = 0; e < kB2; ++e) tap[e] = tp[warp * 2 * R + (it * kB2 + e) * 2 + half];
#pragma unroll
          for (int e = 0; e < kB2; ++e) load_corners(xc, ucin, urs, tap[e].x, c[e]);
#pragma unroll
          for (int e = 0; e < kB2; ++e) {
            if ((tap[e].x & 15) == 0) continue;
            const int j = it * kB2 + e;
            const int row = warp * 2 * R + j * 2 + half;
            const float4 g4 = *reinterpret_cast<const float4*>(gcol + row * kGcolPitch + ul * 64 + q * 4);
            const float lh = __int_as_float(tap[e].y), lw = __int_as_float(tap[e].z), mk = __int_as_float(tap[e].w);
            const float hh = 1.f - lh, hw = 1.f - lw;
            const float w0 = hh * hw, w1 = hh * lw, w2 = lh * hw, w3 = lh * lw;
            const F2 LH = f2_pack(lh, lh), LW = f2_pack(lw, lw), HH = f2_pack(hh, hh), HW = f2_pack(hw, hw);
            const F2 W0 = f2_pack(w0, w0), W1 = f2_pack(w1, w1), W2 = f2_pack(w2, w2), W3 = f2_pack(w3, w3);
            const F2 MK = f2_pack(mk, mk);
            const F2 G[2] = {f2_pack(g4.x, g4.y), f2_pack(g4.z, g4.w)};
            const F2 A0[2] = {f2_pack(c[e].v0.x, c[e].v0.y), f2_pack(c[e].v0.z, c[e].v0.w)};
            const F2 A1[2] = {f2_pack(c[e].v1.x, c[e].v1.y), f2_pack(c[e].v1.z, c[e].v1.w)};
            const F2 A2[2] = {f2_pack(c[e].v2.x, c[e].v2.y), f2_pack(c[e].v2.z, c[e].v2.w)};
            const F2 A3[2] = {f2_pack(c[e].v3.x, c[e].v3.y), f2_pack(c[e].v3.z, c[e].v3.w)};
            F2 GM[2];
            F2 th2 = f2_pack(0.f, 0.f), tw2 = th2, tm2 = th2;
#pragma unroll
            for (int i = 0; i < 2; ++i) {
              GM[i] = f2_mul(G[i], MK);
              const F2 dh = f2_fma(LW, f2_sub(A3[i], A1[i]), f2_mul(HW, f2_sub(A2[i], A0[i])));
              const F2 dw = f2_fma(LH, f2_sub(A3[i], A2[i]), f2_mul(HH, f2_sub(A1[i], A0[i])));
              const F2 val = f2_fma(W3, A3[i], f2_fma(W2, A2[i], f2_fma(W1, A1[i], f2_mul(W0, A0[i]))));
              th2 = f2_fma(GM[i], dh, th2);
              tw2 = f2_fma(GM[i], dw, tw2);
              tm2 = f2_fma(G[i], val, tm2);
            }
            {
              float e0, e1;
              f2_unpack(th2, e0, e1);
              sh[j] += e0 + e1;
              f2_unpack(tw2, e0, e1);
              sw[j] += e0 + e1;
              f2_unpack(tm2, e0, e1);
              sm[j] += e0 + e1;
            }
            if (gimg) {
              float* gp = gc + (uint32_t)(tap[e].x >> 4) * ucin;
              red_add_v4_if(tap[e].x & 1, gp, f2_mul(GM[0], W0), f2_mul(GM[1], W0));
              red_add_v4_if(tap[e].x & 2, gp + ucin, f2_mul(GM[0], W1), f2_mul(GM[1], W1));
              red_add_v4_if(tap[e].x & 4, gp + urs, f2_mul(GM[0], W2), f2_mul(GM[1], W2));
              red_add_v4_if(tap[e].x & 8, gp + (urs + ucin), f2_mul(GM[0], W3), f2_mul(GM[1], W3));
            }
          }
        }
      }
      named_bar_sync(1, kWorkers);
    }
    flush();
  } else if (warp == kWorkerWarps) {
    if (lane == 0) {
      const uint32_t half_bytes = (uint32_t)(split ? 2 : 1) * (uint32_t)kTile;
      int c = 0;
      for (int ml = 0; ml < nm; ++ml) {
        const int m = m0 + ml;
        for (int ks = 0; ks < d.nks; ++ks, ++c) {
          const int s = c & 1;
          const uint32_t par = (uint32_t)((c >> 1) & 1);
          mbar_wait(&empty_bar[s], par ^ 1u);
          mbar_arrive_expect_tx(&full_bar[s], 2 * half_bytes);
          const size_t atile = (((size_t)b * d.tiles_img + pt) * d.SG + sg) * d.nks + ks;
          const size_t btile = ((size_t)sg * d.MC + m) * d.nks + ks;
          bulk_g2s(smem + s * kStage, gt + atile * (size_t)(2 * kTile), half_bytes, &full_bar[s]);
          bulk_g2s(smem + s * kStage + 2 * kTile, wt + btile * (size_t)(2 * kTile), half_bytes, &full_bar[s]);
        }
      }
    }
  }
}

template <int BN>
__device__ __forceinline__ void gw_tile_store(const float (&acc)[BN / 4], float* __restrict__ tile, int pitch) {
#pragma unroll
  for (int i = 0; i < BN / 4; i += 2) red_add_v2(tile + (size_t)acc_row<BN>(i) * pitch + acc_col<BN>(i), acc[i], acc[i + 1]);
}

__global__ void dcn_gw_reduce_kernel(const float* __restrict__ part, const TC d, float* __restrict__ gw) {
  const long long total = (long long)d.SG * d.U * 64 * d.ops;
  const long long idx = (long long)blockIdx.x * blockDim.x + threadIdx.x;
  if (idx >= total) return;
  const int ocl = (int)(idx % d.ops);
  const long long r = idx / d.ops;
  const int rowu = (int)(r % ((long long)d.U * 64)), sg = (int)(r / ((long long)d.U * 64));
  const int u = rowu >> 6, ch = rowu & 63;
  const int kp = u / d.cbs, cb = u - kp * d.cbs;
  const int ec = sg * d.cps + cb * 64 + ch, egrp = ec / d.cpg, ecin = ec - egrp * d.cpg;
  const int oc = sg * d.ops + ocl;
  if (oc / d.opg != egrp) return;
  gw[((size_t)oc * d.cpg + ecin) * d.KK + kp] = __ldg(part + ((size_t)sg * d.MC * 128 + rowu) * d.ops + ocl);
}

constexpr int kRedOc = 16, kRedCh = 16;
__global__ void __launch_bounds__(256) dcn_gw_reduce_tile_kernel(const float* __restrict__ part, const TC d,
                                                                  float* __restrict__ gw) {
  __shared__ float tile[9 * kRedCh][kRedOc + 1];
  const int per_sg = d.cps / kRedCh;
  const int sg = blockIdx.x / per_sg, c0 = (blockIdx.x - sg * per_sg) * kRedCh;
  const int cb = c0 >> 6, ch0 = c0 & 63;
  const int ocl0 = blockIdx.y * kRedOc;
  const int tid = threadIdx.x;
  {
    const int j = tid & (kRedOc - 1), r0 = tid / kRedOc;
    for (int row = r0; row < d.KK * kRedCh; row += 256 / kRedOc) {
      const int kp = row / kRedCh, ch = row - kp * kRedCh;
      tile[row][j] = __ldg(part + ((size_t)sg * d.MC * 128 + (size_t)(kp * d.cbs + cb) * 64 + ch0 + ch) * d.ops + ocl0 + j);
    }
  }
  __syncthreads();
  const int ec0 = sg * d.cps + c0;
  for (int i = tid; i < kRedOc * kRedCh * d.KK; i += 256) {
    const int j = i / (kRedCh * d.KK), e = i - j * (kRedCh * d.KK);
    const int ch = e / d.KK, kp = e - ch * d.KK;
    const int oc = sg * d.ops + ocl0 + j, grp = oc / d.opg;
    const int ec = ec0 + ch;
    if (ec / d.cpg == grp) gw[((size_t)oc * d.cpg + (ec - grp * d.cpg)) * d.KK + kp] = tile[kp * kRedCh + ch][j];
  }
}

template <int BN>
__global__ void __launch_bounds__(kThreads, 1) dcn_bwd_weight_tc_kernel(const float* __restrict__ xh,
                                                                        const float* __restrict__ offset,
                                                                        const float* __restrict__ mask,
                                                                        const uint8_t* __restrict__ gt, const TC d,
                                                                        const K3P k, const int split,
                                                                        float* __restrict__ gw) {
  extern __shared__ uint8_t smem_raw[];
  uint8_t* smem = smem_raw + ((1024u - (smem_u32(smem_raw) & 1023u)) & 1023u);
  int4* tap_s = reinterpret_cast<int4*>(smem + k.S * k.stage_bytes);
  uint64_t* bars = reinterpret_cast<uint64_t*>(reinterpret_cast<uint8_t*>(tap_s) + 4096);
  uint64_t* full_bar = bars;
  uint64_t* empty_bar = bars + k.S;

  const int tid = threadIdx.x, warp = tid >> 5, lane = tid & 31;
  const int mb = blockIdx.y;
  const int sg = blockIdx.x / k.noct, oct = blockIdx.x - sg * k.noct;
  const int total = d.N * d.stages_img;
  const int gs0 = blockIdx.z * k.sper, gs1 = min(total, gs0 + k.sper), ns = gs1 - gs0;

  if (tid == 0) {
    for (int s = 0; s < k.S; ++s) {
      mbar_init(&full_bar[s], kWorkerWarps + 1);
      mbar_init(&empty_bar[s], kWorkerWarps);
    }
    mbar_init_fence();
  }
  __syncthreads();
  if (warp < kWorkerWarps) reg_alloc<kWorkerRegs>();
  else reg_dealloc<kSideRegs>();

  if (warp < kWorkerWarps) {
    const int half = lane >> 4, q = lane & 15;
    const int u = 2 * mb + half;
    const bool u_ok = u < d.U;
    const int kp = u_ok ? u / d.cbs : 0, cb = u_ok ? u - kp * d.cbs : 0;
    const int cbase = sg * d.cps + cb * 64;
    const int dg = cbase / d.cpdg;
    constexpr int PX = 64 / kWorkerWarps;
    const int tl_half = (lane / PX) & 1, tl_j = lane % PX;
    const int tl_u = 2 * mb + tl_half;
    const bool tl_ok = lane < 2 * PX && tl_u < d.U;
    const int tl_kp = tl_ok ? tl_u / d.cbs : 0;
    const int tl_dg = tl_ok ? (sg * d.cps + (tl_u - tl_kp * d.cbs) * 64) / d.cpdg : 0;
    int4* my_taps = tap_s + warp * 2 * (2 * PX);
    auto stage_of = [&](int i, int& b, int& pbase) {
      const int gs = gs0 + i;
      b = gs / d.stages_img;
      pbase = (gs - b * d.stages_img) * 64;
    };
    if (ns > 0) {
      int b0, pb0;
      stage_of(0, b0, pb0);
      if (lane < 2 * PX) my_taps[lane] = tl_ok ? make_tap(d, offset, mask, b0, tl_dg, tl_kp, pb0 + warp * PX + tl_j) : make_int4(0, 0, 0, 0);
    }
    __syncwarp();
    float acc[BN / 4];
#pragma unroll
    for (int i = 0; i < BN / 4; ++i) acc[i] = 0.f;
    auto stage = [&](int i) {
      const int s = i % k.S;
      const uint32_t par = (uint32_t)((i / k.S) & 1);
      int b, pbase, bn = 0, pbn = 0;
      stage_of(i, b, pbase);
      const bool have_next = i + 1 < ns;
      TapRaw raw = {0.f, 0.f, 1.f};
      if (have_next) {
        stage_of(i + 1, bn, pbn);
        if (tl_ok) raw = tap_loads(d, offset, mask, bn, tl_dg, tl_kp, pbn + warp * PX + tl_j);
      }
      const float* __restrict__ xc = xh + ((size_t)b * d.H * d.W - (size_t)(d.W + 1)) * d.Cin + cbase + q * 4;
      const uint32_t ucin = (uint32_t)d.Cin, urs = (uint32_t)(d.W * d.Cin);
      uint8_t* a_hi = smem + s * k.stage_bytes + half * 8192;
      uint8_t* a_lo = a_hi + kTile;
      const int4* cur = my_taps + (i & 1) * (2 * PX) + half * PX;
      mbar_wait(&empty_bar[s], par ^ 1u);
      {
        int4 tap[PX];
        Taps4 c[PX];
#pragma unroll
        for (int j = 0; j < PX; ++j) tap[j] = cur[j];
#pragma unroll
        for (int j = 0; j < PX; ++j) load_corners(xc, ucin, urs, tap[j].x, c[j]);
#pragma unroll
        for (int j = 0; j < PX; ++j) {
          const uint32_t r = (uint32_t)(warp * PX + j);
          gather_store(c[j], tap[j], a_hi, a_lo, swz128(r, (uint32_t)(q >> 1)) + (uint32_t)(q & 1) * 8u, split != 0);
        }
      }
      if (have_next && lane < 2 * PX)
        my_taps[((i + 1) & 1) * (2 * PX) + lane] =
            tl_ok ? tap_finish(d, raw, mask != nullptr, tl_kp, pbn + warp * PX + tl_j) : make_int4(0, 0, 0, 0);
      fence_proxy_async();
      __syncwarp();
      if (lane == 0) mbar_arrive(&full_bar[s]);
      mbar_wait(&full_bar[s], par);
      const uint32_t sa = smem_u32(smem + s * k.stage_bytes), sb = sa + 2 * kTile;
      mma_stage<BN, 1>(acc, sa, sa + kTile, sb, sb + (uint32_t)BN * 128u, split);
    };
    stage(0);
    for (int i = 1; i < ns; ++i) {
      stage(i);
      wgmma_wait<1>();
      __syncwarp();
      if (lane == 0) mbar_arrive(&empty_bar[(i - 1) % k.S]);
    }
    wgmma_wait<0>();
    gw_tile_store<BN>(acc, gw + ((size_t)sg * d.MC * 128 + (size_t)mb * 128) * d.ops + (size_t)oct * k.BN, d.ops);
  } else if (warp == kWorkerWarps) {
    if (lane == 0) {
      const uint32_t bytes = (uint32_t)(split ? 2 : 1) * (uint32_t)k.BN * 128u;
      for (int i = 0; i < ns; ++i) {
        const int s = i % k.S;
        const uint32_t par = (uint32_t)((i / k.S) & 1);
        mbar_wait(&empty_bar[s], par ^ 1u);
        mbar_arrive_expect_tx(&full_bar[s], bytes);
        const size_t tile = ((size_t)(gs0 + i) * d.SG + sg) * k.noct + oct;
        bulk_g2s(smem + s * k.stage_bytes + 2 * kTile, gt + tile * (size_t)(2 * k.BN * 128), bytes, &full_bar[s]);
      }
    }
  }
}

template <int BN>
__global__ void __launch_bounds__(kThreads, 1) dcn_bwd_weight_cols_kernel(const uint8_t* __restrict__ cols,
                                                                          const uint8_t* __restrict__ gt, const TC d,
                                                                          const K3P k, const int S, const int split,
                                                                          float* __restrict__ gw) {
  extern __shared__ uint8_t smem_raw[];
  uint8_t* smem = smem_raw + ((1024u - (smem_u32(smem_raw) & 1023u)) & 1023u);
  uint64_t* bars = reinterpret_cast<uint64_t*>(smem + S * k.stage_bytes);
  uint64_t* full_bar = bars;
  uint64_t* empty_bar = bars + S;

  const int tid = threadIdx.x, warp = tid >> 5, lane = tid & 31;
  const int mb = blockIdx.y;
  const int sg = blockIdx.x / k.noct, oct = blockIdx.x - sg * k.noct;
  const int total = d.N * d.stages_img;
  const int gs0 = blockIdx.z * k.sper, gs1 = min(total, gs0 + k.sper), ns = gs1 - gs0;
  const int nu = (2 * mb + 1 < d.U) ? 2 : 1;

  if (tid == 0) {
    for (int s = 0; s < S; ++s) {
      mbar_init(&full_bar[s], 1);
      mbar_init(&empty_bar[s], kWorkerWarps);
    }
    mbar_init_fence();
  }
  if (nu == 1 && tid < kWorkers) {
    for (int s = 0; s < S; ++s)
      for (int i = tid; i < 2 * 512; i += kWorkers) {
        const int part = i >> 9, w = i & 511;
        reinterpret_cast<uint4*>(smem + s * k.stage_bytes + part * kTile + 8192)[w] = make_uint4(0, 0, 0, 0);
      }
    fence_proxy_async();
  }
  __syncthreads();
  if (warp < kWorkerWarps) reg_alloc<kWorkerRegs>();
  else reg_dealloc<kSideRegs>();

  if (warp < kWorkerWarps) {
    float acc[BN / 4];
#pragma unroll
    for (int i = 0; i < BN / 4; ++i) acc[i] = 0.f;
    auto issue = [&](int i) {
      const int s = i % S;
      mbar_wait(&full_bar[s], (uint32_t)((i / S) & 1));
      const uint32_t sa = smem_u32(smem + s * k.stage_bytes), sb = sa + 2 * kTile;
      mma_stage<BN, 1>(acc, sa, sa + kTile, sb, sb + (uint32_t)BN * 128u, split);
    };
    issue(0);
    for (int i = 1; i < ns; ++i) {
      issue(i);
      wgmma_wait<1>();
      __syncwarp();
      if (lane == 0) mbar_arrive(&empty_bar[(i - 1) % S]);
    }
    wgmma_wait<0>();
    gw_tile_store<BN>(acc, gw + ((size_t)sg * d.MC * 128 + (size_t)mb * 128) * d.ops + (size_t)oct * k.BN, d.ops);
  } else if (warp == kWorkerWarps) {
    if (lane == 0) {
      const uint32_t parts = split ? 2u : 1u;
      const uint32_t tile_bytes = parts * (uint32_t)kTile;
      const uint32_t gbytes = parts * (uint32_t)k.BN * 128u;
      for (int i = 0; i < ns; ++i) {
        const int s = i % S;
        const uint32_t par = (uint32_t)((i / S) & 1);
        const int gs = gs0 + i;
        const int b = gs / d.stages_img, st = gs - b * d.stages_img;
        mbar_wait(&empty_bar[s], par ^ 1u);
        mbar_arrive_expect_tx(&full_bar[s], (uint32_t)nu * parts * 8192u + gbytes);
        uint8_t* stage = smem + s * k.stage_bytes;
        const uint8_t* src =
            cols + ((((size_t)b * d.tiles_img + (st >> 1)) * d.SG + sg) * d.U + 2 * mb) * tile_bytes + (size_t)(st & 1) * 8192;
        for (int ul = 0; ul < nu; ++ul)
          for (uint32_t part = 0; part < parts; ++part)
            bulk_g2s(stage + part * kTile + ul * 8192, src + (size_t)ul * tile_bytes + (size_t)part * kTile, 8192u, &full_bar[s]);
        const size_t tile = ((size_t)gs * d.SG + sg) * k.noct + oct;
        bulk_g2s(stage + 2 * kTile, gt + tile * (size_t)(2 * k.BN * 128), gbytes, &full_bar[s]);
      }
    }
  }
}

__device__ __forceinline__ void split8(const float (&v)[8], uint4& hi, uint4& lo) {
  split2(v[0], v[1], hi.x, lo.x);
  split2(v[2], v[3], hi.y, lo.y);
  split2(v[4], v[5], hi.z, lo.z);
  split2(v[6], v[7], hi.w, lo.w);
}

__device__ __forceinline__ float w_elem(const float* __restrict__ w, const TC& d, int oc, int c, int kp) {
  const int g = c / d.cpg;
  if (oc / d.opg != g) return 0.f;
  return __ldg(w + ((size_t)oc * d.cpg + (c - g * d.cpg)) * d.KK + kp);
}

__global__ void dcn_wtile_fwd_kernel(const float* __restrict__ w, const TC d, int BN, int noct, uint8_t* __restrict__ dst) {
  const long long idx = (long long)blockIdx.x * blockDim.x + threadIdx.x;
  const long long total = (long long)d.SG * noct * d.U * BN * 8;
  if (idx >= total) return;
  const int c16 = (int)(idx & 7);
  const int r = (int)((idx >> 3) % BN);
  const long long tile = idx / (8LL * BN);
  const int u = (int)(tile % d.U);
  const int oct = (int)((tile / d.U) % noct);
  const int sg = (int)(tile / ((long long)d.U * noct));
  const int kp = u / d.cbs, cb = u - kp * d.cbs;
  const int oc = sg * d.ops + oct * BN + r;
  float v[8];
#pragma unroll
  for (int e = 0; e < 8; ++e) v[e] = w_elem(w, d, oc, sg * d.cps + cb * 64 + c16 * 8 + e, kp);
  uint4 hi, lo;
  split8(v, hi, lo);
  uint8_t* base = dst + tile * (size_t)(2 * BN * 128);
  *reinterpret_cast<uint4*>(base + swz128((uint32_t)r, (uint32_t)c16)) = hi;
  *reinterpret_cast<uint4*>(base + BN * 128 + swz128((uint32_t)r, (uint32_t)c16)) = lo;
}

__global__ void dcn_wtile_bwd_kernel(const float* __restrict__ w, const TC d, uint8_t* __restrict__ dst) {
  const long long idx = (long long)blockIdx.x * blockDim.x + threadIdx.x;
  const long long total = (long long)d.SG * d.MC * d.nks * 128 * 8;
  if (idx >= total) return;
  const int c16 = (int)(idx & 7);
  const int r = (int)((idx >> 3) & 127);
  const long long tile = idx >> 10;
  const int ks = (int)(tile % d.nks);
  const int m = (int)((tile / d.nks) % d.MC);
  const int sg = (int)(tile / ((long long)d.nks * d.MC));
  const int u = 2 * m + (r >> 6);
  float v[8];
#pragma unroll
  for (int e = 0; e < 8; ++e) v[e] = 0.f;
  if (u < d.U) {
    const int kp = u / d.cbs, cb = u - kp * d.cbs;
    const int c = sg * d.cps + cb * 64 + (r & 63);
#pragma unroll
    for (int e = 0; e < 8; ++e) v[e] = w_elem(w, d, sg * d.ops + ks * 64 + c16 * 8 + e, c, kp);
  }
  uint4 hi, lo;
  split8(v, hi, lo);
  uint8_t* base = dst + tile * (size_t)(2 * kTile);
  *reinterpret_cast<uint4*>(base + swz128((uint32_t)r, (uint32_t)c16)) = hi;
  *reinterpret_cast<uint4*>(base + kTile + swz128((uint32_t)r, (uint32_t)c16)) = lo;
}

__device__ __forceinline__ float gout_elem(const float* __restrict__ gout, const float* __restrict__ ysaved, const Epi& ep,
                                           size_t idx, int oc) {
  float g = __ldg(gout + idx);
  if (ep.relu && !(__ldg(ysaved + idx) > 0.f)) g = 0.f;
  if (ep.scale) g *= __ldg(ep.scale + oc);
  return g;
}

__global__ void __launch_bounds__(256) dcn_gout_px_tiles_kernel(const float* __restrict__ gout,
                                                                const float* __restrict__ ysaved, const Epi ep, const TC d,
                                                                uint8_t* __restrict__ dst, uint8_t* __restrict__ dst_oc,
                                                                int BN, int noct) {
  __shared__ float t[64][33];
  const long long tile = blockIdx.x;
  const int ks = (int)(tile % d.nks);
  const int sg = (int)((tile / d.nks) % d.SG);
  const int pt = (int)((tile / ((long long)d.nks * d.SG)) % d.tiles_img);
  const int b = (int)(tile / ((long long)d.nks * d.SG * d.tiles_img));
  const int r0 = blockIdx.y * 32;
  const int p0 = pt * 128 + r0, oc0 = sg * d.ops + ks * 64;
  const int tid = threadIdx.x;
#pragma unroll
  for (int i = 0; i < 8; ++i) {
    const int e = tid + i * 256;
    const int o = e >> 5, pp = e & 31;
    const int p = p0 + pp;
    t[o][pp] = p < d.HoWo ? gout_elem(gout, ysaved, ep, ((size_t)b * d.Cout + oc0 + o) * d.HoWo + p, oc0 + o) : 0.f;
  }
  __syncthreads();
  uint8_t* base = dst + tile * (size_t)(2 * kTile);
  {
    const int r = tid >> 3, c16 = tid & 7;
    float v[8];
#pragma unroll
    for (int i = 0; i < 8; ++i) v[i] = t[c16 * 8 + i][r];
    uint4 hi, lo;
    split8(v, hi, lo);
    *reinterpret_cast<uint4*>(base + swz128((uint32_t)(r0 + r), (uint32_t)c16)) = hi;
    *reinterpret_cast<uint4*>(base + kTile + swz128((uint32_t)(r0 + r), (uint32_t)c16)) = lo;
  }
  if (dst_oc) {
    const int o = tid >> 2, ch = tid & 3;
    const int ocs = ks * 64 + o;
    const int oct = ocs / BN, row = ocs - oct * BN;
    const int pglob = pt * 128 + r0;
    const int ps = pglob >> 6, c16 = ((pglob & 63) >> 3) + ch;
    float v[8];
#pragma unroll
    for (int i = 0; i < 8; ++i) v[i] = t[o][ch * 8 + i];
    uint4 hi, lo;
    split8(v, hi, lo);
    if (ps < d.stages_img) {
      const size_t tile_oc = (((size_t)b * d.stages_img + ps) * d.SG + sg) * noct + oct;
      uint8_t* bo = dst_oc + tile_oc * (size_t)(2 * BN * 128);
      *reinterpret_cast<uint4*>(bo + swz128((uint32_t)row, (uint32_t)c16)) = hi;
      *reinterpret_cast<uint4*>(bo + BN * 128 + swz128((uint32_t)row, (uint32_t)c16)) = lo;
    }
  }
}

__global__ void dcn_gout_oc_tiles_kernel(const float* __restrict__ gout, const float* __restrict__ ysaved, const Epi ep,
                                         const TC d, int BN, int noct, uint8_t* __restrict__ dst) {
  const long long idx = (long long)blockIdx.x * blockDim.x + threadIdx.x;
  const long long total = (long long)d.N * d.stages_img * d.SG * noct * BN * 8;
  if (idx >= total) return;
  const int c16 = (int)(idx & 7);
  const int r = (int)((idx >> 3) % BN);
  const long long tile = idx / (8LL * BN);
  const int oct = (int)(tile % noct);
  const int sg = (int)((tile / noct) % d.SG);
  const int ps = (int)((tile / ((long long)noct * d.SG)) % d.stages_img);
  const int b = (int)(tile / ((long long)noct * d.SG * d.stages_img));
  const int oc = sg * d.ops + oct * BN + r;
  const size_t src = ((size_t)b * d.Cout + oc) * d.HoWo;
  float v[8];
#pragma unroll
  for (int e = 0; e < 8; ++e) {
    const int p = ps * 64 + c16 * 8 + e;
    v[e] = p < d.HoWo ? gout_elem(gout, ysaved, ep, src + p, oc) : 0.f;
  }
  uint4 hi, lo;
  split8(v, hi, lo);
  uint8_t* base = dst + tile * (size_t)(2 * BN * 128);
  *reinterpret_cast<uint4*>(base + swz128((uint32_t)r, (uint32_t)c16)) = hi;
  *reinterpret_cast<uint4*>(base + BN * 128 + swz128((uint32_t)r, (uint32_t)c16)) = lo;
}

__global__ void __launch_bounds__(256) nhwc_to_nchw_kernel(const float* __restrict__ src, int C, int HW,
                                                           float* __restrict__ dst) {
  __shared__ float t[64][33];
  const int hw0 = blockIdx.x * 64, c0 = blockIdx.y * 32;
  const float* __restrict__ s = src + (size_t)blockIdx.z * HW * C;
  float* __restrict__ o = dst + (size_t)blockIdx.z * C * HW;
  const int tid = threadIdx.x;
  for (int e = tid; e < 64 * 32; e += 256) {
    const int pp = e >> 5, cc = e & 31;
    t[pp][cc] = (hw0 + pp < HW && c0 + cc < C) ? __ldg(s + (size_t)(hw0 + pp) * C + c0 + cc) : 0.f;
  }
  __syncthreads();
  for (int e = tid; e < 64 * 32; e += 256) {
    const int cc = e >> 6, pp = e & 63;
    if (hw0 + pp < HW && c0 + cc < C) o[(size_t)(c0 + cc) * HW + hw0 + pp] = t[pp][cc];
  }
}

__global__ void dcn_epilogue_kernel(float* __restrict__ y, long long total, int Cout, int HoWo, const Epi ep) {
  const long long i = (long long)blockIdx.x * blockDim.x + threadIdx.x;
  if (i >= total) return;
  const int oc = (int)((i / HoWo) % Cout);
  float v = y[i];
  if (ep.scale) v *= __ldg(ep.scale + oc);
  if (ep.shift) v += __ldg(ep.shift + oc);
  if (ep.relu) v = fmaxf(v, 0.f);
  y[i] = v;
}

int to_nhwc(const float* x, const TC& d, float* dst, cudaStream_t stream) {
  d2b_pyramid P = {};
  P.num_levels = 1;
  P.feat[0] = x;
  P.H[0] = d.H;
  P.W[0] = d.W;
  P.scale[0] = 1.f;
  float* dsts[1] = {dst};
  return d2b_pyramid_nchw_to_nhwc(&P, d.N, d.Cin, dsts, (void*)stream);
}

}

int d2b_deform_conv_tc_supported(const d2b_dcn_params* p) {
  TC d;
  K1P k1;
  return make_tc(p, d) && plan_k1(d, k1);
}

int d2b_deform_conv_tc_bwd_supported(const d2b_dcn_params* p) {
  TC d;
  K2P k2;
  K3P k3;
  return make_tc(p, d) && plan_k2(d, k2) && plan_k3(d, k3);
}

size_t d2b_deform_conv_tc_fwd_workspace(const d2b_dcn_params* p, int x_nhwc) {
  TC d;
  K1P k;
  if (!make_tc(p, d) || !plan_k1(d, k)) return 0;
  size_t b = align256((size_t)d.SG * k.noct * d.U * 2 * k.BN * 128);
  if (!x_nhwc) b += align256(sizeof(float) * (size_t)d.N * d.H * d.W * d.Cin);
  return b;
}

size_t d2b_deform_conv_tc_cols_bytes(const d2b_dcn_params* p, int precision) {
  TC d;
  K1P k;
  if (precision == 0 || !make_tc(p, d) || !plan_k1(d, k)) return 0;
  return (size_t)d.N * d.tiles_img * d.SG * d.U * (size_t)(precision == 1 ? 2 : 1) * kTile;
}

int d2b_deform_conv_forward_tc(const float* x, const float* offset, const float* mask, const float* weight,
                               const float* scale, const float* shift, int relu, const d2b_dcn_params* p, int precision,
                               int tcflags, float* out, void* cols, void* workspace, size_t workspace_bytes, void* stream_) {
  cudaStream_t stream = (cudaStream_t)stream_;
  const int x_nhwc = tcflags & 1;
  TC d;
  K1P k;
  if (!make_tc(p, d) || !plan_k1(d, k)) return D2B_EUNSUPPORTED;
  if (d.N == 0) return D2B_OK;
  if (tcflags & 2) {
    if (mask) return D2B_EINVAL;
    mask = use_fused_offset_mask(d, offset);
  }
  if (!workspace || workspace_bytes < d2b_deform_conv_tc_fwd_workspace(p, x_nhwc)) return D2B_EWORKSPACE;
  if ((reinterpret_cast<uintptr_t>(workspace) & 255) || (x_nhwc && (reinterpret_cast<uintptr_t>(x) & 15)) ||
      (reinterpret_cast<uintptr_t>(cols) & 15))
    return D2B_EINVAL;
  uint8_t* ws = reinterpret_cast<uint8_t*>(workspace);
  uint8_t* wt = ws;
  ws += align256((size_t)d.SG * k.noct * d.U * 2 * k.BN * 128);
  const float* xh = x;
  if (!x_nhwc) {
    float* xn = reinterpret_cast<float*>(ws);
    int rc = to_nhwc(x, d, xn, stream);
    if (rc) return rc;
    xh = xn;
  }
  {
    const long long total = (long long)d.SG * k.noct * d.U * k.BN * 8;
    dcn_wtile_fwd_kernel<<<d2b_cdiv(total, 256), 256, 0, stream>>>(weight, d, k.BN, k.noct, wt);
    D2B_CHECK_LAUNCH();
  }
  K1P kc;
  bool colfed = false;
  if (cols && k.noct > 1) {
    K1P k1;
    if (plan_k1(d, k1, true) && plan_k1c(d, k1, kc)) {
      k = k1;
      colfed = true;
    }
  }
  if (k.red) D2B_CUDA(cudaMemsetAsync(out, 0, sizeof(float) * (size_t)d.N * d.Cout * d.HoWo, stream));
  const int smem_bytes = k.S * k.stage_bytes + k.tap_bytes + 1024 + 128;
  const int split = precision == 1 ? 1 : 0;
  const Epi ep = {scale, shift, relu};
  dim3 grid(d.N * d.tiles_img, d.SG * k.goct, k.ksplit);
#define D2B_LAUNCH_K1(BN)                                                                                              \
  {                                                                                                                    \
    D2B_ALLOW_BIG_SMEM(dcn_fwd_tc_kernel<BN>);                                                                         \
    dcn_fwd_tc_kernel<BN><<<grid, kThreads, smem_bytes, stream>>>(xh, offset, mask, wt, ep, d, k, split, out,        \
                                                                    reinterpret_cast<uint8_t*>(cols));                 \
  }
  if (k.BN == 16) D2B_LAUNCH_K1(16)
  else if (k.BN == 32) D2B_LAUNCH_K1(32)
  else if (k.BN == 64) D2B_LAUNCH_K1(64)
  else D2B_LAUNCH_K1(128)
#undef D2B_LAUNCH_K1
  D2B_CHECK_LAUNCH();
  if (colfed) {
    const int smem_c = kc.S * kc.stage_bytes + 1024 + 128;
    dim3 grid_c(d.N * d.tiles_img * kc.goct, d.SG, kc.ksplit);
    const uint8_t* cl = reinterpret_cast<const uint8_t*>(cols);
#define D2B_LAUNCH_K1C(BN)                                                                                             \
  {                                                                                                                    \
    D2B_ALLOW_BIG_SMEM(dcn_fwd_cols_kernel<BN>);                                                                       \
    dcn_fwd_cols_kernel<BN><<<grid_c, kThreads, smem_c, stream>>>(cl, wt, ep, d, kc, split, out);                      \
  }
    if (kc.BN == 16) D2B_LAUNCH_K1C(16)
    else if (kc.BN == 32) D2B_LAUNCH_K1C(32)
    else if (kc.BN == 64) D2B_LAUNCH_K1C(64)
    else D2B_LAUNCH_K1C(128)
#undef D2B_LAUNCH_K1C
    D2B_CHECK_LAUNCH();
  }
  if (k.red && (scale || relu)) {
    const long long total = (long long)d.N * d.Cout * d.HoWo;
    dcn_epilogue_kernel<<<d2b_cdiv(total, 256), 256, 0, stream>>>(out, total, d.Cout, d.HoWo, ep);
    D2B_CHECK_LAUNCH();
  }
  return D2B_OK;
}

size_t d2b_deform_conv_tc_bwd_workspace(const d2b_dcn_params* p, int x_nhwc, int need_data, int need_weight) {
  TC d;
  K2P k2;
  K3P k3;
  if (!make_tc(p, d) || !plan_k2(d, k2) || !plan_k3(d, k3)) return 0;
  size_t b = 0;
  const size_t xbytes = align256(sizeof(float) * (size_t)d.N * d.H * d.W * d.Cin);
  if (!x_nhwc) b += xbytes;
  if (need_data && !x_nhwc) b += xbytes;
  if (need_data) {
    b += align256((size_t)d.N * d.tiles_img * d.SG * d.nks * 2 * kTile);
    b += align256((size_t)d.SG * d.MC * d.nks * 2 * kTile);
  }
  if (need_weight) {
    b += align256((size_t)d.N * d.stages_img * d.SG * k3.noct * 2 * k3.BN * 128);
    b += align256(sizeof(float) * (size_t)d.SG * d.MC * 128 * d.ops);
  }
  return b;
}

int d2b_deform_conv_backward_tc(const float* x, const float* offset, const float* mask, const float* weight,
                                const float* grad_out, const float* scale, const float* y_saved, int relu,
                                const d2b_dcn_params* p, int precision, int tcflags, const void* cols, float* grad_x,
                                float* grad_offset, float* grad_mask, float* grad_weight, void* workspace,
                                size_t workspace_bytes, void* stream_) {
  cudaStream_t stream = (cudaStream_t)stream_;
  const int x_nhwc = tcflags & 1;
  TC d;
  K2P k2;
  K3P k3;
  if (!make_tc(p, d) || !plan_k2(d, k2) || !plan_k3(d, k3)) return D2B_EUNSUPPORTED;
  const int need_data = (grad_x || grad_offset || grad_mask) ? 1 : 0, need_weight = grad_weight ? 1 : 0;
  const bool fused_om = (tcflags & 2) != 0;
  if (fused_om && (mask || grad_mask)) return D2B_EINVAL;
  if (relu && !y_saved) return D2B_EINVAL;
  const size_t nx = (size_t)d.N * d.H * d.W * d.Cin, noff = (size_t)d.N * d.DG * (fused_om ? 3 : 2) * d.KK * d.HoWo;
  const size_t nm = (size_t)d.N * d.DG * d.KK * d.HoWo, nw = (size_t)d.Cout * d.cpg * d.KK;
  if (fused_om) {
    mask = use_fused_offset_mask(d, offset);
    if (grad_offset) grad_mask = grad_offset + (size_t)d.DG * 2 * d.KK * d.HoWo;
  }
  const Epi ep = {scale, nullptr, relu};
  if (d.N == 0 || (!need_data && !need_weight)) {
    void* zp[3] = {grad_offset, fused_om ? nullptr : grad_mask, grad_weight};
    size_t zb[3] = {noff * 4, nm * 4, nw * 4};
    return d2b_zero_buffers(zp, zb, 3, stream);
  }
  if (!workspace || workspace_bytes < d2b_deform_conv_tc_bwd_workspace(p, x_nhwc, need_data, need_weight)) return D2B_EWORKSPACE;
  if ((reinterpret_cast<uintptr_t>(workspace) & 255) || (x_nhwc && (reinterpret_cast<uintptr_t>(x) & 15)) ||
      (x_nhwc && grad_x && (reinterpret_cast<uintptr_t>(grad_x) & 15)) || (reinterpret_cast<uintptr_t>(cols) & 15))
    return D2B_EINVAL;
  const int split = precision == 1 ? 1 : 0;
  uint8_t* ws = reinterpret_cast<uint8_t*>(workspace);
  const size_t xbytes = align256(sizeof(float) * nx);
  const float* xh = x;
  if (!x_nhwc) {
    float* xn = reinterpret_cast<float*>(ws);
    ws += xbytes;
    int rc = to_nhwc(x, d, xn, stream);
    if (rc) return rc;
    xh = xn;
  }
  float* gxh = nullptr;
  if (need_data && grad_x) gxh = x_nhwc ? grad_x : reinterpret_cast<float*>(ws);
  uint8_t* gt_px = nullptr;
  uint8_t* wt = nullptr;
  if (need_data) {
    if (!x_nhwc) ws += xbytes;
    gt_px = ws;
    ws += align256((size_t)d.N * d.tiles_img * d.SG * d.nks * 2 * kTile);
    wt = ws;
    ws += align256((size_t)d.SG * d.MC * d.nks * 2 * kTile);
  }
  uint8_t* gt_oc = need_weight ? ws : nullptr;
  float* gw_part = nullptr;
  if (need_weight) {
    ws += align256((size_t)d.N * d.stages_img * d.SG * k3.noct * 2 * k3.BN * 128);
    gw_part = reinterpret_cast<float*>(ws);
  }
  {
    void* zp[4] = {grad_offset, fused_om ? nullptr : grad_mask, gxh, gw_part};
    size_t zb[4] = {noff * 4, nm * 4, nx * 4, sizeof(float) * (size_t)d.SG * d.MC * 128 * d.ops};
    int rc = d2b_zero_buffers(zp, zb, 4, stream);
    if (rc) return rc;
  }
  if (need_data) {
    dcn_gout_px_tiles_kernel<<<dim3((unsigned)((size_t)d.N * d.tiles_img * d.SG * d.nks), 4), 256, 0, stream>>>(
        grad_out, y_saved, ep, d, gt_px, gt_oc, k3.BN, k3.noct);
    D2B_CHECK_LAUNCH();
    {
      const long long total = (long long)d.SG * d.MC * d.nks * 128 * 8;
      dcn_wtile_bwd_kernel<<<d2b_cdiv(total, 256), 256, 0, stream>>>(weight, d, wt);
      D2B_CHECK_LAUNCH();
    }
    const int smem_bytes = 2 * 4 * kTile + 128 * kGcolPitch * 4 + k2.tap_bytes + 1024 + 128;
    D2B_ALLOW_BIG_SMEM(dcn_bwd_data_tc_kernel);
    dim3 grid(d.N * d.tiles_img, d.SG, k2.msplit);
    dcn_bwd_data_tc_kernel<<<grid, kThreads, smem_bytes, stream>>>(xh, offset, mask, gt_px, wt, d, k2, split, gxh, grad_offset,
                                                                  mask ? grad_mask : nullptr);
    D2B_CHECK_LAUNCH();
    if (grad_x && !x_nhwc) {
      dim3 g2(d2b_cdiv(d.H * d.W, 64), d2b_cdiv(d.Cin, 32), d.N);
      nhwc_to_nchw_kernel<<<g2, 256, 0, stream>>>(gxh, d.Cin, d.H * d.W, grad_x);
      D2B_CHECK_LAUNCH();
    }
  }
  if (need_weight) {
    if (!need_data) {
      const long long total = (long long)d.N * d.stages_img * d.SG * k3.noct * k3.BN * 8;
      dcn_gout_oc_tiles_kernel<<<d2b_cdiv(total, 256), 256, 0, stream>>>(grad_out, y_saved, ep, d, k3.BN, k3.noct, gt_oc);
      D2B_CHECK_LAUNCH();
    }
    dim3 grid(d.SG * k3.noct, d.MC, k3.nsplit);
    if (cols) {
      const int S = std::min(6, (kMaxSmem - 2048) / k3.stage_bytes);
      const int smem_bytes = S * k3.stage_bytes + 1024 + 128;
      const uint8_t* cl = reinterpret_cast<const uint8_t*>(cols);
#define D2B_LAUNCH_K3C(BN)                                                                                             \
  {                                                                                                                      \
    D2B_ALLOW_BIG_SMEM(dcn_bwd_weight_cols_kernel<BN>);                                                                \
    dcn_bwd_weight_cols_kernel<BN><<<grid, kThreads, smem_bytes, stream>>>(cl, gt_oc, d, k3, S, split, gw_part);       \
  }
      if (k3.BN == 64) D2B_LAUNCH_K3C(64)
      else D2B_LAUNCH_K3C(128)
#undef D2B_LAUNCH_K3C
    } else {
      const int smem_bytes = k3.S * k3.stage_bytes + 4096 + 1024 + 128;
#define D2B_LAUNCH_K3(BN)                                                                                              \
  {                                                                                                                      \
    D2B_ALLOW_BIG_SMEM(dcn_bwd_weight_tc_kernel<BN>);                                                                  \
    dcn_bwd_weight_tc_kernel<BN><<<grid, kThreads, smem_bytes, stream>>>(xh, offset, mask, gt_oc, d, k3, split, gw_part); \
  }
      if (k3.BN == 64) D2B_LAUNCH_K3(64)
      else D2B_LAUNCH_K3(128)
#undef D2B_LAUNCH_K3
    }
    D2B_CHECK_LAUNCH();
    {
      if (d.KK <= 9) {
        dcn_gw_reduce_tile_kernel<<<dim3(d.SG * (d.cps / kRedCh), d.ops / kRedOc), 256, 0, stream>>>(gw_part, d, grad_weight);
      } else {
        const long long total = (long long)d.SG * d.U * 64 * d.ops;
        dcn_gw_reduce_kernel<<<d2b_cdiv(total, 256), 256, 0, stream>>>(gw_part, d, grad_weight);
      }
      D2B_CHECK_LAUNCH();
    }
  }
  return D2B_OK;
}
```

detectron2_b200/csrc/deform_conv_tc.cuh:

```cuda
#pragma once
#include <stddef.h>

#include "../../include/d2b200.h"

int d2b_deform_conv_tc_supported(const d2b_dcn_params* p);
int d2b_deform_conv_tc_bwd_supported(const d2b_dcn_params* p);

size_t d2b_deform_conv_tc_fwd_workspace(const d2b_dcn_params* p, int x_nhwc);
size_t d2b_deform_conv_tc_cols_bytes(const d2b_dcn_params* p, int precision);
size_t d2b_deform_conv_tc_bwd_workspace(const d2b_dcn_params* p, int x_nhwc, int need_data, int need_weight);

int d2b_deform_conv_forward_tc(const float* x, const float* offset, const float* mask, const float* weight,
                               const float* scale, const float* shift, int relu, const d2b_dcn_params* p, int precision,
                               int tcflags, float* out, void* cols, void* workspace, size_t workspace_bytes, void* stream);
int d2b_deform_conv_backward_tc(const float* x, const float* offset, const float* mask, const float* weight,
                                const float* grad_out, const float* scale, const float* y_saved, int relu,
                                const d2b_dcn_params* p, int precision, int tcflags, const void* cols, float* grad_x,
                                float* grad_offset, float* grad_mask, float* grad_weight, void* workspace,
                                size_t workspace_bytes, void* stream);
```

detectron2_b200/csrc/tc_common.cuh:

```cuda
#pragma once
#include <cuda_bf16.h>
#include <stdint.h>

namespace d2b_tc {

__device__ __forceinline__ uint32_t smem_u32(const void* p) { return (uint32_t)__cvta_generic_to_shared(p); }

__device__ __forceinline__ void mbar_init(uint64_t* bar, uint32_t count) {
  asm volatile("mbarrier.init.shared::cta.b64 [%0], %1;" ::"r"(smem_u32(bar)), "r"(count));
}
__device__ __forceinline__ void mbar_init_fence() { asm volatile("fence.mbarrier_init.release.cluster;" ::: "memory"); }
__device__ __forceinline__ void mbar_arrive(uint64_t* bar) {
  asm volatile("mbarrier.arrive.shared::cta.b64 _, [%0];" ::"r"(smem_u32(bar)) : "memory");
}
__device__ __forceinline__ void mbar_arrive_expect_tx(uint64_t* bar, uint32_t bytes) {
  asm volatile("mbarrier.arrive.expect_tx.shared::cta.b64 _, [%0], %1;" ::"r"(smem_u32(bar)), "r"(bytes) : "memory");
}
__device__ __forceinline__ bool mbar_try_wait(uint64_t* bar, uint32_t parity) {
  uint32_t ok;
  asm volatile(
      "{\n\t"
      ".reg .pred p;\n\t"
      "mbarrier.test_wait.parity.shared::cta.b64 p, [%1], %2;\n\t"
      "selp.u32 %0, 1, 0, p;\n\t"
      "}"
      : "=r"(ok)
      : "r"(smem_u32(bar)), "r"(parity)
      : "memory");
  return ok != 0;
}
__device__ __forceinline__ uint64_t global_timer_ns() {
  uint64_t t;
  asm volatile("mov.u64 %0, %%globaltimer;" : "=l"(t));
  return t;
}
__device__ __forceinline__ void mbar_wait(uint64_t* bar, uint32_t parity) {
  if (mbar_try_wait(bar, parity)) return;
  const uint64_t t0 = global_timer_ns();
  for (uint32_t spin = 1;; ++spin) {
    if (mbar_try_wait(bar, parity)) return;
    if ((spin & 1023u) == 0 && global_timer_ns() - t0 > 2000000000ull) __trap();
  }
}

__device__ __forceinline__ void fence_proxy_async() { asm volatile("fence.proxy.async.shared::cta;" ::: "memory"); }
__device__ __forceinline__ void named_bar_sync(uint32_t id, uint32_t nthreads) {
  asm volatile("bar.sync %0, %1;" ::"r"(id), "r"(nthreads) : "memory");
}

__device__ __forceinline__ void bulk_g2s(void* smem_dst, const void* gmem_src, uint32_t bytes, uint64_t* bar) {
  asm volatile("cp.async.bulk.shared::cluster.global.mbarrier::complete_tx::bytes [%0], [%1], %2, [%3];" ::"r"(smem_u32(smem_dst)),
               "l"(gmem_src), "r"(bytes), "r"(smem_u32(bar))
               : "memory");
}
__device__ __forceinline__ void bulk_s2g(void* gmem_dst, const void* smem_src, uint32_t bytes) {
  asm volatile("cp.async.bulk.global.shared::cta.bulk_group [%0], [%1], %2;" ::"l"(gmem_dst), "r"(smem_u32(smem_src)), "r"(bytes)
               : "memory");
}
__device__ __forceinline__ void bulk_commit() { asm volatile("cp.async.bulk.commit_group;" ::: "memory"); }
__device__ __forceinline__ void bulk_wait_read0() { asm volatile("cp.async.bulk.wait_group.read 0;" ::: "memory"); }
__device__ __forceinline__ void bulk_wait0() { asm volatile("cp.async.bulk.wait_group 0;" ::: "memory"); }

__device__ __forceinline__ uint64_t wgmma_desc(uint32_t smem_addr, uint32_t lbo_bytes, uint32_t sbo_bytes) {
  uint64_t d = 0;
  d |= (uint64_t)((smem_addr >> 4) & 0x3FFF);
  d |= (uint64_t)((lbo_bytes >> 4) & 0x3FFF) << 16;
  d |= (uint64_t)((sbo_bytes >> 4) & 0x3FFF) << 32;
  d |= (uint64_t)1 << 62;
  return d;
}
__device__ __forceinline__ void wgmma_fence() { asm volatile("wgmma.fence.sync.aligned;" ::: "memory"); }
__device__ __forceinline__ void wgmma_commit() { asm volatile("wgmma.commit_group.sync.aligned;" ::: "memory"); }
template <int kPending>
__device__ __forceinline__ void wgmma_wait() { asm volatile("wgmma.wait_group.sync.aligned %0;" ::"n"(kPending) : "memory"); }

template <int N, int kTransA>
struct Wgmma;

template <int kTransA>
struct Wgmma<8, kTransA> {
  __device__ __forceinline__ static void mma(float (&d)[4], uint64_t a, uint64_t b, int accumulate) {
    asm volatile(
        "{\n\t.reg .pred p;\n\tsetp.ne.b32 p, %4, 0;\n\t"
        "wgmma.mma_async.sync.aligned.m64n8k16.f32.bf16.bf16 {%0, %1, %2, %3}, %5, %6, p, 1, 1, %7, 0;\n\t}"
        : "+f"(d[0]), "+f"(d[1]), "+f"(d[2]), "+f"(d[3])
        : "r"(accumulate), "l"(a), "l"(b), "n"(kTransA));
  }
};
template <int kTransA>
struct Wgmma<16, kTransA> {
  __device__ __forceinline__ static void mma(float (&d)[8], uint64_t a, uint64_t b, int accumulate) {
    asm volatile(
        "{\n\t.reg .pred p;\n\tsetp.ne.b32 p, %8, 0;\n\t"
        "wgmma.mma_async.sync.aligned.m64n16k16.f32.bf16.bf16 {%0, %1, %2, %3, %4, %5, %6, %7}, %9, %10, p, 1, 1, %11, 0;\n\t}"
        : "+f"(d[0]), "+f"(d[1]), "+f"(d[2]), "+f"(d[3]), "+f"(d[4]), "+f"(d[5]), "+f"(d[6]), "+f"(d[7])
        : "r"(accumulate), "l"(a), "l"(b), "n"(kTransA));
  }
};
template <int kTransA>
struct Wgmma<32, kTransA> {
  __device__ __forceinline__ static void mma(float (&d)[16], uint64_t a, uint64_t b, int accumulate) {
    asm volatile(
        "{\n\t.reg .pred p;\n\tsetp.ne.b32 p, %16, 0;\n\t"
        "wgmma.mma_async.sync.aligned.m64n32k16.f32.bf16.bf16 {%0, %1, %2, %3, %4, %5, %6, %7, %8, %9, %10, %11, %12, %13, %14, %15}, %17, %18, p, 1, 1, %19, 0;\n\t}"
        : "+f"(d[0]), "+f"(d[1]), "+f"(d[2]), "+f"(d[3]), "+f"(d[4]), "+f"(d[5]), "+f"(d[6]), "+f"(d[7]), "+f"(d[8]), "+f"(d[9]), "+f"(d[10]), "+f"(d[11]), "+f"(d[12]), "+f"(d[13]), "+f"(d[14]), "+f"(d[15])
        : "r"(accumulate), "l"(a), "l"(b), "n"(kTransA));
  }
};
template <int kTransA>
struct Wgmma<64, kTransA> {
  __device__ __forceinline__ static void mma(float (&d)[32], uint64_t a, uint64_t b, int accumulate) {
    asm volatile(
        "{\n\t.reg .pred p;\n\tsetp.ne.b32 p, %32, 0;\n\t"
        "wgmma.mma_async.sync.aligned.m64n64k16.f32.bf16.bf16 {%0, %1, %2, %3, %4, %5, %6, %7, %8, %9, %10, %11, %12, %13, %14, %15, %16, %17, %18, %19, %20, %21, %22, %23, %24, %25, %26, %27, %28, %29, %30, %31}, %33, %34, p, 1, 1, %35, 0;\n\t}"
        : "+f"(d[0]), "+f"(d[1]), "+f"(d[2]), "+f"(d[3]), "+f"(d[4]), "+f"(d[5]), "+f"(d[6]), "+f"(d[7]), "+f"(d[8]), "+f"(d[9]), "+f"(d[10]), "+f"(d[11]), "+f"(d[12]), "+f"(d[13]), "+f"(d[14]), "+f"(d[15]), "+f"(d[16]), "+f"(d[17]), "+f"(d[18]), "+f"(d[19]), "+f"(d[20]), "+f"(d[21]), "+f"(d[22]), "+f"(d[23]), "+f"(d[24]), "+f"(d[25]), "+f"(d[26]), "+f"(d[27]), "+f"(d[28]), "+f"(d[29]), "+f"(d[30]), "+f"(d[31])
        : "r"(accumulate), "l"(a), "l"(b), "n"(kTransA));
  }
};
template <int kTransA>
struct Wgmma<128, kTransA> {
  __device__ __forceinline__ static void mma(float (&d)[64], uint64_t a, uint64_t b, int accumulate) {
    asm volatile(
        "{\n\t.reg .pred p;\n\tsetp.ne.b32 p, %64, 0;\n\t"
        "wgmma.mma_async.sync.aligned.m64n128k16.f32.bf16.bf16 {%0, %1, %2, %3, %4, %5, %6, %7, %8, %9, %10, %11, %12, %13, %14, %15, %16, %17, %18, %19, %20, %21, %22, %23, %24, %25, %26, %27, %28, %29, %30, %31, %32, %33, %34, %35, %36, %37, %38, %39, %40, %41, %42, %43, %44, %45, %46, %47, %48, %49, %50, %51, %52, %53, %54, %55, %56, %57, %58, %59, %60, %61, %62, %63}, %65, %66, p, 1, 1, %67, 0;\n\t}"
        : "+f"(d[0]), "+f"(d[1]), "+f"(d[2]), "+f"(d[3]), "+f"(d[4]), "+f"(d[5]), "+f"(d[6]), "+f"(d[7]), "+f"(d[8]), "+f"(d[9]), "+f"(d[10]), "+f"(d[11]), "+f"(d[12]), "+f"(d[13]), "+f"(d[14]), "+f"(d[15]), "+f"(d[16]), "+f"(d[17]), "+f"(d[18]), "+f"(d[19]), "+f"(d[20]), "+f"(d[21]), "+f"(d[22]), "+f"(d[23]), "+f"(d[24]), "+f"(d[25]), "+f"(d[26]), "+f"(d[27]), "+f"(d[28]), "+f"(d[29]), "+f"(d[30]), "+f"(d[31]), "+f"(d[32]), "+f"(d[33]), "+f"(d[34]), "+f"(d[35]), "+f"(d[36]), "+f"(d[37]), "+f"(d[38]), "+f"(d[39]), "+f"(d[40]), "+f"(d[41]), "+f"(d[42]), "+f"(d[43]), "+f"(d[44]), "+f"(d[45]), "+f"(d[46]), "+f"(d[47]), "+f"(d[48]), "+f"(d[49]), "+f"(d[50]), "+f"(d[51]), "+f"(d[52]), "+f"(d[53]), "+f"(d[54]), "+f"(d[55]), "+f"(d[56]), "+f"(d[57]), "+f"(d[58]), "+f"(d[59]), "+f"(d[60]), "+f"(d[61]), "+f"(d[62]), "+f"(d[63])
        : "r"(accumulate), "l"(a), "l"(b), "n"(kTransA));
  }
};

template <int kRegs>
__device__ __forceinline__ void reg_alloc() { asm volatile("setmaxnreg.inc.sync.aligned.u32 %0;" ::"n"(kRegs)); }
template <int kRegs>
__device__ __forceinline__ void reg_dealloc() { asm volatile("setmaxnreg.dec.sync.aligned.u32 %0;" ::"n"(kRegs)); }

__device__ __forceinline__ void red_add_v4(float* p, float a, float b, float c, float d) {
  asm volatile("red.global.add.v4.f32 [%0], {%1, %2, %3, %4};" ::"l"(p), "f"(a), "f"(b), "f"(c), "f"(d) : "memory");
}
__device__ __forceinline__ void red_add_v2(float* p, float a, float b) {
  asm volatile("red.global.add.v2.f32 [%0], {%1, %2};" ::"l"(p), "f"(a), "f"(b) : "memory");
}
__device__ __forceinline__ void red_add(float* p, float a) {
  asm volatile("red.global.add.f32 [%0], %1;" ::"l"(p), "f"(a) : "memory");
}
__device__ __forceinline__ uint32_t pack_bf16(float a, float b) {
  __nv_bfloat162 v = __floats2bfloat162_rn(a, b);
  return *reinterpret_cast<uint32_t*>(&v);
}
__device__ __forceinline__ void split2(float a, float b, uint32_t& hi, uint32_t& lo) {
  hi = pack_bf16(a, b);
  const float ha = __uint_as_float(hi << 16), hb = __uint_as_float(hi & 0xffff0000u);
  lo = pack_bf16(a - ha, b - hb);
}
__device__ __forceinline__ void split4(const float (&v)[4], uint2& hi, uint2& lo) {
  split2(v[0], v[1], hi.x, lo.x);
  split2(v[2], v[3], hi.y, lo.y);
}
struct F2 {
  float x, y;
};
__device__ __forceinline__ F2 f2_pack(float a, float b) { return F2{a, b}; }
__device__ __forceinline__ void f2_unpack(F2 p, float& a, float& b) {
  a = p.x;
  b = p.y;
}
__device__ __forceinline__ F2 f2_fma(F2 w, F2 v, F2 c) { return F2{__fmaf_rn(w.x, v.x, c.x), __fmaf_rn(w.y, v.y, c.y)}; }
__device__ __forceinline__ F2 f2_mul(F2 a, F2 b) { return F2{__fmul_rn(a.x, b.x), __fmul_rn(a.y, b.y)}; }
__device__ __forceinline__ F2 f2_add(F2 a, F2 b) { return F2{__fadd_rn(a.x, b.x), __fadd_rn(a.y, b.y)}; }
__device__ __forceinline__ F2 f2_sub(F2 a, F2 b) { return F2{__fsub_rn(a.x, b.x), __fsub_rn(a.y, b.y)}; }
__device__ __forceinline__ void red_add_v4(float* p, F2 ab, F2 cd) {
  float a, b, c, d;
  f2_unpack(ab, a, b);
  f2_unpack(cd, c, d);
  red_add_v4(p, a, b, c, d);
}
__device__ __forceinline__ void red_add_v4_if(int pred, float* p, F2 ab, F2 cd) {
  float a, b, c, d;
  f2_unpack(ab, a, b);
  f2_unpack(cd, c, d);
  asm volatile(
      "{\n\t.reg .pred q;\n\tsetp.ne.b32 q, %5, 0;\n\t@q red.global.add.v4.f32 [%0], {%1, %2, %3, %4};\n\t}" ::"l"(p),
      "f"(a), "f"(b), "f"(c), "f"(d), "r"(pred)
      : "memory");
}

__device__ __forceinline__ uint32_t swz128(uint32_t r, uint32_t c16) { return r * 128u + ((c16 ^ (r & 7u)) << 4); }

}
```

include/d2b200.h:

```cpp
#ifndef D2B200_H_
#define D2B200_H_

#include <stddef.h>
#include <stdint.h>

#ifdef __cplusplus
extern "C" {
#endif

#define D2B_OK 0
#define D2B_EINVAL (-1)
#define D2B_EWORKSPACE (-2)
#define D2B_EUNSUPPORTED (-3)

#define D2B_ABI_VERSION 4
int d2b_abi_version(void);
int d2b_cuda_version(void);
const char* d2b_arch(void);

int d2b_roi_align_forward(const float* input, int N, int C, int H, int W, const float* rois, int K,
                          float spatial_scale, int pooled_h, int pooled_w, int sampling_ratio,
                          int aligned, float* out, void* stream);
int d2b_roi_align_backward(const float* grad_out, const float* rois, int K, float spatial_scale,
                           int pooled_h, int pooled_w, int N, int C, int H, int W,
                           int sampling_ratio, int aligned, float* grad_in, void* stream);

#define D2B_MAX_LEVELS 8
typedef struct {
  int num_levels;
  const float* feat[D2B_MAX_LEVELS];
  float* grad[D2B_MAX_LEVELS];
  int H[D2B_MAX_LEVELS], W[D2B_MAX_LEVELS];
  float scale[D2B_MAX_LEVELS];
  int min_level, max_level, canonical_level;
  float canonical_box_size;
  const float* level_rois;
} d2b_pyramid;
int d2b_roi_pooler_forward(const d2b_pyramid* pyr, int N, int C, const float* rois, int K, int pooled_h,
                           int pooled_w, int sampling_ratio, int aligned, float* out, void* stream);
int d2b_roi_pooler_backward(const d2b_pyramid* pyr, int N, int C, const float* grad_out, const float* rois,
                            int K, int pooled_h, int pooled_w, int sampling_ratio, int aligned, void* stream);

int d2b_roi_align_forward_nhwc(const float* input, int N, int C, int H, int W, const float* rois, int K,
                               float spatial_scale, int pooled_h, int pooled_w, int sampling_ratio,
                               int aligned, float* out, void* stream);
int d2b_roi_pooler_forward_nhwc(const d2b_pyramid* pyr, int N, int C, const float* rois, int K, int pooled_h,
                                int pooled_w, int sampling_ratio, int aligned, float* out, void* stream);
int d2b_pyramid_nchw_to_nhwc(const d2b_pyramid* pyr, int N, int C, float* const* dst, void* stream);
int d2b_pyramid_nhwc_to_nchw(const d2b_pyramid* pyr, int N, int C, float* const* dst, void* stream);
#define D2B_F32 0
#define D2B_F16 1
#define D2B_BF16 2
int d2b_pyramid_nchw_to_nhwc_t(const d2b_pyramid* pyr, int N, int C, float* const* dst, int src_dtype, void* stream);
int d2b_pyramid_nhwc_to_nchw_t(const d2b_pyramid* pyr, int N, int C, void* const* dst, int dst_dtype, void* stream);
int d2b_roi_pooler_forward_nhwc_t(const d2b_pyramid* pyr, int N, int C, const float* rois, int K, int pooled_h,
                                  int pooled_w, int sampling_ratio, int aligned, void* out, int out_dtype, void* stream);
int d2b_roi_pooler_backward_nhwc_t(const d2b_pyramid* pyr, int N, int C, const void* grad_out, int grad_dtype,
                                   const float* rois, int K, int pooled_h, int pooled_w, int sampling_ratio, int aligned,
                                   void* stream);
int d2b_roi_align_backward_nhwc(const float* grad_out, const float* rois, int K, float spatial_scale,
                                int pooled_h, int pooled_w, int N, int C, int H, int W,
                                int sampling_ratio, int aligned, float* grad_in, void* stream);
int d2b_roi_pooler_backward_nhwc(const d2b_pyramid* pyr, int N, int C, const float* grad_out, const float* rois,
                                 int K, int pooled_h, int pooled_w, int sampling_ratio, int aligned, void* stream);

int d2b_roi_align_rotated_forward(const float* input, int N, int C, int H, int W, const float* rois,
                                  int K, float spatial_scale, int pooled_h, int pooled_w,
                                  int sampling_ratio, float* out, void* stream);
int d2b_roi_align_rotated_backward(const float* grad_out, const float* rois, int K,
                                   float spatial_scale, int pooled_h, int pooled_w, int N, int C,
                                   int H, int W, int sampling_ratio, float* grad_in, void* stream);
int d2b_roi_align_rotated_forward_nhwc(const float* input, int N, int C, int H, int W, const float* rois,
                                       int K, float spatial_scale, int pooled_h, int pooled_w,
                                       int sampling_ratio, float* out, void* stream);
int d2b_roi_align_rotated_backward_nhwc(const float* grad_out, const float* rois, int K,
                                        float spatial_scale, int pooled_h, int pooled_w, int N, int C,
                                        int H, int W, int sampling_ratio, float* grad_in, void* stream);

int d2b_roi_pooler_rotated_forward(const d2b_pyramid* pyr, int N, int C, const float* rois, int K, int pooled_h,
                                   int pooled_w, int sampling_ratio, float* out, void* stream);
int d2b_roi_pooler_rotated_backward(const d2b_pyramid* pyr, int N, int C, const float* grad_out, const float* rois,
                                    int K, int pooled_h, int pooled_w, int sampling_ratio, void* stream);
int d2b_roi_pooler_rotated_forward_nhwc_t(const d2b_pyramid* pyr, int N, int C, const float* rois, int K, int pooled_h,
                                          int pooled_w, int sampling_ratio, void* out, int out_dtype, void* stream);
int d2b_roi_pooler_rotated_backward_nhwc_t(const d2b_pyramid* pyr, int N, int C, const void* grad_out, int grad_dtype,
                                           const float* rois, int K, int pooled_h, int pooled_w, int sampling_ratio,
                                           void* stream);

#define D2B_ROI_ROTATED 1
#define D2B_ROI_BACKWARD 2
int d2b_roi_pooler_nhwc_supported(const d2b_pyramid* pyr, int C, int pooled_h, int pooled_w, int flags);

#define D2B_NMS_ROTATED 1
#define D2B_NMS_NO_OFFSET 2
size_t d2b_nms_workspace_bytes(int64_t M, int flags, int64_t max_segment);
int d2b_nms(const float* boxes, const float* scores, const int64_t* idxs, int64_t M,
            double iou_threshold, int flags, int64_t max_segment, int64_t* keep, int64_t* num_keep,
            void* workspace, size_t workspace_bytes, void* stream);

typedef struct {
  int num_levels;
  const float* proposals[D2B_MAX_LEVELS];
  const int64_t* topk_idx[D2B_MAX_LEVELS];
  const float* topk_scores[D2B_MAX_LEVELS];
  int A[D2B_MAX_LEVELS], k[D2B_MAX_LEVELS];
} d2b_rpn_levels;
int d2b_rpn_prepare(const d2b_rpn_levels* lv, int N, const float* image_hw, float min_box_size, int use_offsets,
                    float* flat_boxes, float* nms_boxes, float* nms_scores, float* raw_scores, int64_t* cat_ids,
                    int* nonfinite, void* stream);
int d2b_rpn_select(const int64_t* keep, const int64_t* num_keep, int N, int T, int post_nms_topk,
                   const float* flat_boxes, const float* raw_scores, const int64_t* cat_ids, float* out_boxes,
                   float* out_scores, int64_t* out_index, int64_t* counts, void* stream);

#define D2B_MAX_IMAGES 64
typedef struct {
  int num_levels;
  const float* anchors[D2B_MAX_LEVELS];
  const float* deltas[D2B_MAX_LEVELS];
  const int64_t* topk_idx[D2B_MAX_LEVELS];
  const float* topk_scores[D2B_MAX_LEVELS];
  int R[D2B_MAX_LEVELS], k[D2B_MAX_LEVELS];
} d2b_dense_levels;
int d2b_frcnn_prepare(const float* boxes, const float* scores, const int* row_start, int N, int num_classes, int kreg,
                      const float* image_hw, float score_thresh, int cap, float* cand_boxes, float* nms_boxes,
                      float* nms_scores, float* raw_scores, int64_t* cand_flat, int64_t* cat_ids, int64_t* n_cand,
                      int64_t* row_map, void* stream);
int d2b_dense_prepare(const d2b_dense_levels* lv, int N, int num_classes, const float* weights, float scale_clamp,
                      float* flat_boxes, float* nms_boxes, float* nms_scores, float* raw_scores, int64_t* classes,
                      int64_t* cat_ids, void* stream);

int d2b_rrpn_prepare(const d2b_rpn_levels* lv, int N, const float* image_hw, float min_box_size, int seg_per_image,
                     float* flat_boxes, float* nms_boxes, float* nms_scores, float* raw_scores, int64_t* cat_ids,
                     int* nonfinite, void* stream);
int d2b_frcnn_rotated_prepare(const float* boxes, const float* scores, const int* row_start, int N, int num_classes,
                              int kreg, const float* image_hw, float score_thresh, int cap, int seg_per_image,
                              float* cand_boxes, float* nms_boxes, float* nms_scores, float* raw_scores, int64_t* cand_flat,
                              int64_t* cat_ids, int64_t* n_cand, int64_t* row_map, void* stream);
int d2b_rpn_select_rotated(const int64_t* keep, const int64_t* num_keep, int N, int T, int post_nms_topk,
                           const float* flat_boxes, const float* raw_scores, const int64_t* cat_ids, float* out_boxes,
                           float* out_scores, int64_t* out_index, int64_t* counts, void* stream);

#define D2B_MATCH_ROTATED 1
#define D2B_MATCH_LOW_QUALITY 2
#define D2B_MATCH_APPEND_GT 4
#define D2B_MATCH_MAX_THRESHOLDS 8
#define D2B_MATCH_STATUS_INVALID_IOU 1
size_t d2b_match_workspace_bytes(int N, int Gmax, int P);
int d2b_match_boxes(const float* gt_boxes, const int64_t* gt_count, int N, int Gmax, const float* pred_boxes,
                    int64_t pred_image_stride, const int64_t* pred_count, int Pmax, const double* thresholds,
                    int num_thresholds, const int* labels, int flags, const float* image_hw, double boundary_thresh,
                    const int64_t* gt_classes, int64_t num_classes, int64_t* matches, int8_t* match_labels,
                    float* matched_gt_boxes, int64_t* classes, int* status, void* workspace, size_t workspace_bytes,
                    void* stream);

#define D2B_SAMPLE_MAX_SAMPLES 8192
size_t d2b_sample_labels_workspace_bytes(int N, int P, int num_samples);
int d2b_sample_labels(const void* labels, int label_kind, int N, int P, int64_t bg_label, int num_samples, int max_pos,
                      const uint64_t* seed, int8_t* out_labels, int64_t* sampled, int64_t* num_pos, int64_t* num_neg,
                      void* workspace, size_t workspace_bytes, void* stream);

int d2b_mask_loss_forward(const float* logits, int K, int C, int S, const uint8_t* gt_masks, int G, int H, int W,
                          const float* boxes, const int64_t* mask_index, const int64_t* classes,
                          float* loss_per_roi, uint8_t* targets, void* stream);
int d2b_mask_loss_backward(const float* logits, int K, int C, int S, const uint8_t* targets, const int64_t* classes,
                           const float* grad_scale, float* grad_logits, void* stream);

#define D2B_KEYPOINTS_MAX_S 241
size_t d2b_keypoints_workspace_bytes(int R, int K);
int d2b_keypoints_from_heatmaps(const float* maps, int R, int K, int S, const float* rois, float* out, void* workspace,
                                size_t workspace_bytes, void* stream);

int d2b_keypoint_loss_forward(const void* logits, int dtype, int N, int K, int S, const float* keypoints,
                              const float* boxes, int64_t* target, uint8_t* valid, float* loss_per_kp, int64_t* num_valid,
                              void* stream);
int d2b_keypoint_loss_backward(const void* logits, int dtype, int N, int K, int S, const int64_t* target,
                               const uint8_t* valid, const float* grad_scale, void* grad_logits, void* stream);

#define D2B_LABELS_I8 0
#define D2B_LABELS_I64 1
#define D2B_LOSS_STATUS_INVALID_BOX 1
#define D2B_LOSS_STATUS_INVALID_CLASS 2
#define D2B_LOSS_STATUS_INVALID_BOX_ORDER 4
#define D2B_LOSS_SMOOTH_L1 0
#define D2B_LOSS_GIOU 1
typedef struct {
  int num_levels;
  const void* logits[D2B_MAX_LEVELS];
  const void* deltas[D2B_MAX_LEVELS];
  void* grad_logits[D2B_MAX_LEVELS];
  void* grad_deltas[D2B_MAX_LEVELS];
  int R[D2B_MAX_LEVELS];
} d2b_dense_loss_levels;
size_t d2b_dense_loss_workspace_bytes(const d2b_dense_loss_levels* lv, int N, int K, int dtype);
int d2b_dense_loss_forward(const d2b_dense_loss_levels* lv, int N, int K, int box_dim, int dtype, const float* anchors,
                           const float* gt_boxes, const void* labels, int label_kind, float gamma, float alpha, float beta,
                           int loss_type, float scale_clamp, const float* weights, float* cls_sum, float* reg_sum, int64_t* num_pos, int64_t* num_neg,
                           int* status, void* workspace, size_t workspace_bytes, void* stream);
int d2b_dense_loss_backward(const d2b_dense_loss_levels* lv, int N, int K, int box_dim, int dtype, const float* anchors,
                            const float* gt_boxes, const void* labels, int label_kind, float gamma, float alpha, float beta,
                            int loss_type, float scale_clamp, const float* weights, const float* grad_cls, const float* grad_reg, void* stream);
size_t d2b_frcnn_loss_workspace_bytes(int R);
int d2b_frcnn_loss_forward(const void* scores, const void* deltas, int R, int K, int kreg, int box_dim, int dtype,
                           const float* proposals, const float* gt_boxes, const int64_t* gt_classes, float beta,
                           int loss_type, float scale_clamp, const float* weights, float* cls_sum, float* reg_sum, int64_t* num_fg, int64_t* num_accurate,
                           int64_t* fg_num_accurate, int64_t* num_false_negative, int* status, void* workspace,
                           size_t workspace_bytes, void* stream);
int d2b_frcnn_loss_backward(const void* scores, const void* deltas, int R, int K, int kreg, int box_dim, int dtype,
                            const float* proposals, const float* gt_boxes, const int64_t* gt_classes, float beta,
                            int loss_type, float scale_clamp, const float* weights, const float* grad_cls, const float* grad_reg, void* grad_scores,
                            void* grad_deltas, void* stream);

int d2b_box_iou_rotated(const float* boxes1, int64_t N, const float* boxes2, int64_t M, float* ious,
                        void* stream);

typedef struct {
  int N, Cin, H, W, Cout, kh, kw, stride_h, stride_w, pad_h, pad_w, dil_h, dil_w, groups,
      deformable_groups;
} d2b_dcn_params;

#define D2B_DCN_X_NHWC 1
int d2b_deform_conv_tc_shape_supported(const d2b_dcn_params* p, int backward);
size_t d2b_deform_conv_forward_workspace_bytes(const d2b_dcn_params* p, int precision, int flags);
size_t d2b_deform_conv_cols_bytes(const d2b_dcn_params* p, int precision);
int d2b_deform_conv_forward(const float* x, const float* offset, const float* mask,
                            const float* weight, const float* bias, const d2b_dcn_params* p,
                            int precision, int flags, float* out, void* cols, void* workspace,
                            size_t workspace_bytes, void* stream);
size_t d2b_deform_conv_backward_workspace_bytes(const d2b_dcn_params* p, int precision, int flags, int need_data,
                                                int need_weight);
int d2b_deform_conv_backward(const float* x, const float* offset, const float* mask,
                             const float* weight, const float* grad_out, const d2b_dcn_params* p,
                             int precision, int flags, const void* cols, float* grad_x, float* grad_offset,
                             float* grad_mask, float* grad_weight, float* grad_bias, void* workspace,
                             size_t workspace_bytes, void* stream);

int d2b_deform_conv_fused_forward(const float* x, const float* offset_mask, const float* weight, const float* scale,
                                  const float* shift, int relu, const d2b_dcn_params* p, int precision, int flags,
                                  float* out, void* cols, void* workspace, size_t workspace_bytes, void* stream);
int d2b_deform_conv_fused_backward(const float* x, const float* offset_mask, const float* weight, const float* scale,
                                   int relu, const float* y, const float* grad_out, const d2b_dcn_params* p,
                                   int precision, int flags, const void* cols, float* grad_x, float* grad_offset_mask,
                                   float* grad_weight, void* workspace, size_t workspace_bytes, void* stream);

int d2b_paste_masks(const float* masks, const float* boxes, int N, int M, int H, int W,
                    float threshold, uint8_t* out, void* stream);
int d2b_paste_masks_packed(const float* masks, const float* boxes, int N, int M, int H, int W,
                           float threshold, uint32_t* out, void* stream);

#ifdef __cplusplus
}
#endif
#endif
```

Before: 285.7.

## Fuse deformable conv backward data and weight gradients into one wgmma kernel

Adds a fused backward kernel that computes the column gradient and the weight gradient in a single pass. Both wgmma products share the staged grad_out tiles, and the bilinear scatter runs in the same kernel, so the separate weight-gradient kernel is skipped when the fused path applies. The scatter math is moved into a shared helper, and the Wgmma wrappers gain a transpose-B option. The cost is a more complex warp-specialised kernel with higher shared-memory use, which limits it to output-channel groups of 64 or 128.

```diff
diff --git a/detectron2_b200/_C.py b/detectron2_b200/_C.py
--- a/detectron2_b200/_C.py
+++ b/detectron2_b200/_C.py
@@ -121,6 +121,7 @@
         "d2b_sample_labels_workspace_bytes": (sz, [i, i, i]),
         "d2b_sample_labels": (i, [vp, i, i, i, i64, i, i, vp, vp, i64p, i64p, i64p, vp, sz, vp]),
         "d2b_deform_conv_tc_shape_supported": (i, [C.POINTER(DcnParams), i]),
+        "d2b_deform_conv_tc_bwd_path": (i, [C.POINTER(DcnParams), i, i, i]),
         "d2b_deform_conv_forward_workspace_bytes": (sz, [C.POINTER(DcnParams), i, i]),
         "d2b_deform_conv_cols_bytes": (sz, [C.POINTER(DcnParams), i]),
         "d2b_deform_conv_forward": (i, [f32p, f32p, f32p, f32p, f32p, C.POINTER(DcnParams), i, i, f32p, vp, vp, sz, vp]),
diff --git a/detectron2_b200/csrc/deform_conv.cu b/detectron2_b200/csrc/deform_conv.cu
--- a/detectron2_b200/csrc/deform_conv.cu
+++ b/detectron2_b200/csrc/deform_conv.cu
@@ -339,6 +339,10 @@
   return backward ? d2b_deform_conv_tc_bwd_supported(p) : d2b_deform_conv_tc_supported(p);
 }
 
+D2B_API int d2b_deform_conv_tc_bwd_path(const d2b_dcn_params* p, int has_cols, int need_data, int need_weight) {
+  return d2b_deform_conv_tc_bwd_kernels(p, has_cols, need_data, need_weight);
+}
+
 D2B_API size_t d2b_deform_conv_forward_workspace_bytes(const d2b_dcn_params* p, int precision, int flags) {
   if (precision == 0) return 0;
   if (precision == -1 && !d2b_deform_conv_tc_supported(p)) return 0;
diff --git a/detectron2_b200/csrc/deform_conv_tc.cu b/detectron2_b200/csrc/deform_conv_tc.cu
--- a/detectron2_b200/csrc/deform_conv_tc.cu
+++ b/detectron2_b200/csrc/deform_conv_tc.cu
@@ -171,6 +171,33 @@
   return k.S >= 2;
 }
 
+struct K2FP { int sper, nsplit, ntab, stage_bytes; };
+
+__host__ __device__ inline void unit_kp_dg(const TC& d, int sg, int u, int& kp, int& dg) {
+  kp = u / d.cbs;
+  dg = (sg * d.cps + (u - kp * d.cbs) * 64) / d.cpdg;
+}
+
+int k2f_smem(const TC& d, const K2FP& k) { return d.nks * 2 * kTile + 2 * k.stage_bytes + 64 * 128 * 4 + k.ntab * 64 * 16 + 64 + 1024; }
+
+bool plan_k2f(const TC& d, K2FP& k) {
+  if (d.ops != 64 && d.ops != 128) return false;
+  k.ntab = 1;
+  for (int sg = 0; sg < d.SG; ++sg)
+    for (int u = 0; u + 1 < d.U; u += 2) {
+      int kp0, dg0, kp1, dg1;
+      unit_kp_dg(d, sg, u, kp0, dg0);
+      unit_kp_dg(d, sg, u + 1, kp1, dg1);
+      if (kp0 != kp1 || dg0 != dg1) k.ntab = 2;
+    }
+  k.stage_bytes = d.nks * 2 * 8192 + 2 * 2 * 8192;
+  const int total = d.N * d.stages_img;
+  k.nsplit = best_split((long long)d.SG * d.MC, total, std::min(total, 4 * d2b_num_sms()), 3);
+  k.sper = d2b_cdiv(total, k.nsplit);
+  k.nsplit = d2b_cdiv(total, k.sper);
+  return k2f_smem(d, k) <= kMaxSmem;
+}
+
 struct TapRaw {
   float oh, ow, m;
 };
@@ -498,6 +525,49 @@
   }
 }
 
+__device__ __forceinline__ void scatter_tap(const Taps4& c, int4 tap, float4 g4, float* gc, uint32_t ucin, uint32_t urs,
+                                            float& sh, float& sw, float& sm) {
+  const float lh = __int_as_float(tap.y), lw = __int_as_float(tap.z), mk = __int_as_float(tap.w);
+  const float hh = 1.f - lh, hw = 1.f - lw;
+  const float w0 = hh * hw, w1 = hh * lw, w2 = lh * hw, w3 = lh * lw;
+  const F2 LH = f2_pack(lh, lh), LW = f2_pack(lw, lw), HH = f2_pack(hh, hh), HW = f2_pack(hw, hw);
+  const F2 W0 = f2_pack(w0, w0), W1 = f2_pack(w1, w1), W2 = f2_pack(w2, w2), W3 = f2_pack(w3, w3);
+  const F2 MK = f2_pack(mk, mk);
+  const F2 G[2] = {f2_pack(g4.x, g4.y), f2_pack(g4.z, g4.w)};
+  const F2 A0[2] = {f2_pack(c.v0.x, c.v0.y), f2_pack(c.v0.z, c.v0.w)};
+  const F2 A1[2] = {f2_pack(c.v1.x, c.v1.y), f2_pack(c.v1.z, c.v1.w)};
+  const F2 A2[2] = {f2_pack(c.v2.x, c.v2.y), f2_pack(c.v2.z, c.v2.w)};
+  const F2 A3[2] = {f2_pack(c.v3.x, c.v3.y), f2_pack(c.v3.z, c.v3.w)};
+  F2 GM[2];
+  F2 th2 = f2_pack(0.f, 0.f), tw2 = th2, tm2 = th2;
+#pragma unroll
+  for (int i = 0; i < 2; ++i) {
+    GM[i] = f2_mul(G[i], MK);
+    const F2 dh = f2_fma(LW, f2_sub(A3[i], A1[i]), f2_mul(HW, f2_sub(A2[i], A0[i])));
+    const F2 dw = f2_fma(LH, f2_sub(A3[i], A2[i]), f2_mul(HH, f2_sub(A1[i], A0[i])));
+    const F2 val = f2_fma(W3, A3[i], f2_fma(W2, A2[i], f2_fma(W1, A1[i], f2_mul(W0, A0[i]))));
+    th2 = f2_fma(GM[i], dh, th2);
+    tw2 = f2_fma(GM[i], dw, tw2);
+    tm2 = f2_fma(G[i], val, tm2);
+  }
+  {
+    float e0, e1;
+    f2_unpack(th2, e0, e1);
+    sh += e0 + e1;
+    f2_unpack(tw2, e0, e1);
+    sw += e0 + e1;
+    f2_unpack(tm2, e0, e1);
+    sm += e0 + e1;
+  }
+  if (gc) {
+    float* gp = gc + (uint32_t)(tap.x >> 4) * ucin;
+    red_add_v4_if(tap.x & 1, gp, f2_mul(GM[0], W0), f2_mul(GM[1], W0));
+    red_add_v4_if(tap.x & 2, gp + ucin, f2_mul(GM[0], W1), f2_mul(GM[1], W1));
+    red_add_v4_if(tap.x & 4, gp + urs, f2_mul(GM[0], W2), f2_mul(GM[1], W2));
+    red_add_v4_if(tap.x & 8, gp + (urs + ucin), f2_mul(GM[0], W3), f2_mul(GM[1], W3));
+  }
+}
+
 __global__ void __launch_bounds__(kThreads, 1) dcn_bwd_data_tc_kernel(const float* __restrict__ xh,
                                                                       const float* __restrict__ offset,
                                                                       const float* __restrict__ mask,
@@ -650,46 +720,8 @@
             if ((tap[e].x & 15) == 0) continue;
             const int j = it * kB2 + e;
             const int row = warp * 2 * R + j * 2 + half;
-            const float4 g4 = *reinterpret_cast<const float4*>(gcol + row * kGcolPitch + ul * 64 + q * 4);
-            const float lh = __int_as_float(tap[e].y), lw = __int_as_float(tap[e].z), mk = __int_as_float(tap[e].w);
-            const float hh = 1.f - lh, hw = 1.f - lw;
-            const float w0 = hh * hw, w1 = hh * lw, w2 = lh * hw, w3 = lh * lw;
-            const F2 LH = f2_pack(lh, lh), LW = f2_pack(lw, lw), HH = f2_pack(hh, hh), HW = f2_pack(hw, hw);
-            const F2 W0 = f2_pack(w0, w0), W1 = f2_pack(w1, w1), W2 = f2_pack(w2, w2), W3 = f2_pack(w3, w3);
-            const F2 MK = f2_pack(mk, mk);
-            const F2 G[2] = {f2_pack(g4.x, g4.y), f2_pack(g4.z, g4.w)};
-            const F2 A0[2] = {f2_pack(c[e].v0.x, c[e].v0.y), f2_pack(c[e].v0.z, c[e].v0.w)};
-            const F2 A1[2] = {f2_pack(c[e].v1.x, c[e].v1.y), f2_pack(c[e].v1.z, c[e].v1.w)};
-            const F2 A2[2] = {f2_pack(c[e].v2.x, c[e].v2.y), f2_pack(c[e].v2.z, c[e].v2.w)};
-            const F2 A3[2] = {f2_pack(c[e].v3.x, c[e].v3.y), f2_pack(c[e].v3.z, c[e].v3.w)};
-            F2 GM[2];
-            F2 th2 = f2_pack(0.f, 0.f), tw2 = th2, tm2 = th2;
-#pragma unroll
-            for (int i = 0; i < 2; ++i) {
-              GM[i] = f2_mul(G[i], MK);
-              const F2 dh = f2_fma(LW, f2_sub(A3[i], A1[i]), f2_mul(HW, f2_sub(A2[i], A0[i])));
-              const F2 dw = f2_fma(LH, f2_sub(A3[i], A2[i]), f2_mul(HH, f2_sub(A1[i], A0[i])));
-              const F2 val = f2_fma(W3, A3[i], f2_fma(W2, A2[i], f2_fma(W1, A1[i], f2_mul(W0, A0[i]))));
-              th2 = f2_fma(GM[i], dh, th2);
-              tw2 = f2_fma(GM[i], dw, tw2);
-              tm2 = f2_fma(G[i], val, tm2);
-            }
-            {
-              float e0, e1;
-              f2_unpack(th2, e0, e1);
-              sh[j] += e0 + e1;
-              f2_unpack(tw2, e0, e1);
-              sw[j] += e0 + e1;
-              f2_unpack(tm2, e0, e1);
-              sm[j] += e0 + e1;
-            }
-            if (gimg) {
-              float* gp = gc + (uint32_t)(tap[e].x >> 4) * ucin;
-              red_add_v4_if(tap[e].x & 1, gp, f2_mul(GM[0], W0), f2_mul(GM[1], W0));
-              red_add_v4_if(tap[e].x & 2, gp + ucin, f2_mul(GM[0], W1), f2_mul(GM[1], W1));
-              red_add_v4_if(tap[e].x & 4, gp + urs, f2_mul(GM[0], W2), f2_mul(GM[1], W2));
-              red_add_v4_if(tap[e].x & 8, gp + (urs + ucin), f2_mul(GM[0], W3), f2_mul(GM[1], W3));
-            }
+            scatter_tap(c[e], tap[e], *reinterpret_cast<const float4*>(gcol + row * kGcolPitch + ul * 64 + q * 4),
+                        gimg ? gc : nullptr, ucin, urs, sh[j], sw[j], sm[j]);
           }
         }
       }
@@ -969,6 +1001,245 @@
   }
 }
 
+
+template <int kSplit>
+__device__ __forceinline__ void mma_gcol_(float (&acc)[16], uint32_t a_hi, uint32_t a_lo, uint32_t b_hi, uint32_t b_lo) {
+  const uint32_t bo = (uint32_t)(threadIdx.x >> 7) * 32u * 128u;
+  wgmma_fence();
+#pragma unroll
+  for (int kk = 0; kk < 4; ++kk) {
+    const uint32_t ak = (uint32_t)kk * 32u, bk = bo + (uint32_t)kk * 32u;
+    Wgmma<32, 0>::mma(acc, wgmma_desc(a_hi + ak, 0, 1024), wgmma_desc(b_hi + bk, 0, 1024), 1);
+    if (kSplit) {
+      Wgmma<32, 0>::mma(acc, wgmma_desc(a_hi + ak, 0, 1024), wgmma_desc(b_lo + bk, 0, 1024), 1);
+      Wgmma<32, 0>::mma(acc, wgmma_desc(a_lo + ak, 0, 1024), wgmma_desc(b_hi + bk, 0, 1024), 1);
+    }
+  }
+  wgmma_commit();
+}
+
+template <int BN, int kSplit>
+__device__ __forceinline__ void mma_gw_(float (&acc)[BN / 4], uint32_t a_hi, uint32_t a_lo, uint32_t b_hi, uint32_t b_lo) {
+  const int g = threadIdx.x >> 7;
+  const uint32_t ao = (uint32_t)(g & 1) * 8192u;
+  const uint32_t n0 = (uint32_t)(g >> 1) * (uint32_t)(BN / 2);
+  const uint32_t bo = (n0 >> 6) * 8192u + (n0 & 63u) * 2u;
+  wgmma_fence();
+#pragma unroll
+  for (int kk = 0; kk < 4; ++kk) {
+    const uint32_t ak = ao + (uint32_t)kk * 2048u, bk = bo + (uint32_t)kk * 2048u;
+    Wgmma<BN / 2, 1, 1>::mma(acc, wgmma_desc(a_hi + ak, 8192, 1024), wgmma_desc(b_hi + bk, 8192, 1024), 1);
+    if (kSplit) {
+      Wgmma<BN / 2, 1, 1>::mma(acc, wgmma_desc(a_hi + ak, 8192, 1024), wgmma_desc(b_lo + bk, 8192, 1024), 1);
+      Wgmma<BN / 2, 1, 1>::mma(acc, wgmma_desc(a_lo + ak, 8192, 1024), wgmma_desc(b_hi + bk, 8192, 1024), 1);
+    }
+  }
+  wgmma_commit();
+}
+
+__device__ __forceinline__ int gcol_idx(int row, int col) { return row * 128 + (col ^ ((row & 7) << 3)); }
+
+template <int BN>
+__global__ void __launch_bounds__(kThreads, 1) dcn_bwd_fused_tc_kernel(const float* __restrict__ xh,
+                                                                       const float* __restrict__ offset,
+                                                                       const float* __restrict__ mask,
+                                                                       const uint8_t* __restrict__ gt,
+                                                                       const uint8_t* __restrict__ wt,
+                                                                       const uint8_t* __restrict__ cols, const TC d,
+                                                                       const K2FP k, const int split,
+                                                                       float* __restrict__ gxh, float* __restrict__ goff,
+                                                                       float* __restrict__ gmask, float* __restrict__ gw) {
+  constexpr int NKS = BN / 64;
+  extern __shared__ uint8_t smem_raw[];
+  uint8_t* smem = smem_raw + ((1024u - (smem_u32(smem_raw) & 1023u)) & 1023u);
+  uint8_t* wres = smem;
+  uint8_t* stg = smem + NKS * 2 * kTile;
+  float* gcol = reinterpret_cast<float*>(stg + 2 * k.stage_bytes);
+  int4* taps = reinterpret_cast<int4*>(gcol + 64 * 128);
+  uint64_t* bars = reinterpret_cast<uint64_t*>(taps + k.ntab * 64);
+  uint64_t* full_bar = bars;
+  uint64_t* empty_bar = bars + 2;
+  uint64_t* w_bar = bars + 4;
+
+  const int tid = threadIdx.x, warp = tid >> 5, lane = tid & 31;
+  const int sg = blockIdx.x / d.MC, m = blockIdx.x - sg * d.MC;
+  const int total = d.N * d.stages_img;
+  const int gs0 = blockIdx.y * k.sper, ns = min(total, gs0 + k.sper) - gs0;
+  const int nu = (2 * m + 1 < d.U) ? 2 : 1;
+  int kpa, dga, kpb, dgb;
+  unit_kp_dg(d, sg, 2 * m, kpa, dga);
+  unit_kp_dg(d, sg, 2 * m + nu - 1, kpb, dgb);
+  const int ntab = (kpa != kpb || dga != dgb) ? 2 : 1;
+
+  if (tid == 0) {
+    for (int s = 0; s < 2; ++s) {
+      mbar_init(&full_bar[s], 1);
+      mbar_init(&empty_bar[s], kWorkerWarps);
+    }
+    mbar_init(w_bar, 1);
+    mbar_init_fence();
+  }
+  if (nu == 1 && tid < kWorkers) {
+    for (int s = 0; s < 2; ++s)
+      for (int i = tid; i < 2 * 512; i += kWorkers) {
+        const int part = i >> 9, w = i & 511;
+        reinterpret_cast<uint4*>(stg + s * k.stage_bytes + NKS * 16384 + part * 16384 + 8192)[w] = make_uint4(0, 0, 0, 0);
+      }
+    fence_proxy_async();
+  }
+  __syncthreads();
+  if (warp < kWorkerWarps) reg_alloc<kWorkerRegs>();
+  else reg_dealloc<kSideRegs>();
+
+  if (warp < kWorkerWarps) {
+    const int half = lane >> 4, q = lane & 15;
+    const uint32_t ucin = (uint32_t)d.Cin, urs = (uint32_t)(d.W * d.Cin);
+    constexpr int R = 64 / (2 * kWorkerWarps);
+    float sh[R], sw[R], sm[R];
+#pragma unroll
+    for (int j = 0; j < R; ++j) sh[j] = sw[j] = sm[j] = 0.f;
+    float wacc[BN / 4];
+#pragma unroll
+    for (int i = 0; i < BN / 4; ++i) wacc[i] = 0.f;
+
+    auto flush = [&](int tab, int kp, int dg, int b, int p0) {
+      const bool b8 = q & 8, b4 = q & 4, b2 = q & 2;
+      const float v6[6] = {sh[0], sw[0], sm[0], sh[1], sw[1], sm[1]};
+      float v4[4];
+#pragma unroll
+      for (int i = 0; i < 3; ++i) {
+        const float keep = b8 ? v6[i + 3] : v6[i], send = b8 ? v6[i] : v6[i + 3];
+        v4[i] = keep + __shfl_xor_sync(0xffffffffu, send, 8);
+      }
+      v4[3] = 0.f;
+      float v2[2];
+#pragma unroll
+      for (int i = 0; i < 2; ++i) {
+        const float keep = b4 ? v4[i + 2] : v4[i], send = b4 ? v4[i] : v4[i + 2];
+        v2[i] = keep + __shfl_xor_sync(0xffffffffu, send, 4);
+      }
+      float v = (b2 ? v2[1] : v2[0]) + __shfl_xor_sync(0xffffffffu, b2 ? v2[0] : v2[1], 2);
+      v += __shfl_xor_sync(0xffffffffu, v, 1);
+      const int which = (q >> 1) & 3, row = warp * 2 * R + (q >> 3) * 2 + half, p = p0 + row;
+      if (!(q & 1) && which < 3 && p < d.HoWo) {
+        if (which < 2) {
+          if (goff) red_add(goff + (size_t)b * d.off_bs + ((size_t)dg * 2 * d.KK + 2 * kp + which) * d.HoWo + p, v);
+        } else if (gmask) {
+          if (d.mask_sigmoid) {
+            const float mk = __int_as_float(taps[tab * 64 + row].w);
+            v *= mk * (1.f - mk);
+          }
+          red_add(gmask + (size_t)b * d.mask_bs + ((size_t)dg * d.KK + kp) * d.HoWo + p, v);
+        }
+      }
+#pragma unroll
+      for (int j = 0; j < R; ++j) sh[j] = sw[j] = sm[j] = 0.f;
+    };
+
+    const uint32_t sw0 = smem_u32(wres);
+    const int tk = tid < 64 ? 0 : 1, tkp = tk ? kpb : kpa, tdg = tk ? dgb : dga;
+    const bool tbuild = tid < ntab * 64;
+    auto step_of = [&](int i, int& b, int& p0) {
+      b = (gs0 + i) / d.stages_img;
+      p0 = (gs0 + i - b * d.stages_img) * 64;
+    };
+    mbar_wait(w_bar, 0u);
+    if (ns > 0) {
+      int b, p0;
+      step_of(0, b, p0);
+      if (tbuild) taps[tid] = make_tap(d, offset, mask, b, tdg, tkp, p0 + (tid & 63));
+    }
+    for (int i = 0; i < ns; ++i) {
+      const int s = i & 1;
+      int b, p0, bn = 0, pn = 0;
+      step_of(i, b, p0);
+      const bool next = i + 1 < ns;
+      if (next) step_of(i + 1, bn, pn);
+      const uint32_t sgo = smem_u32(stg + s * k.stage_bytes), sco = sgo + NKS * 16384;
+      mbar_wait(&full_bar[s], (uint32_t)((i >> 1) & 1));
+      {
+        float acc[16];
+#pragma unroll
+        for (int e = 0; e < 16; ++e) acc[e] = 0.f;
+#pragma unroll
+        for (int ks = 0; ks < NKS; ++ks) {
+          const uint32_t a = sgo + ks * 8192, bw = sw0 + ks * 2 * kTile;
+          if (split) mma_gcol_<1>(acc, a, a + NKS * 8192, bw, bw + kTile);
+          else mma_gcol_<0>(acc, a, a + NKS * 8192, bw, bw + kTile);
+        }
+        wgmma_wait<0>();
+        const int t = tid & 127;
+#pragma unroll
+        for (int e = 0; e < 16; e += 2) {
+          const int row = (t >> 5) * 16 + ((t & 31) >> 2) + ((e >> 1) & 1) * 8;
+          const int col = (tid >> 7) * 32 + (e >> 2) * 8 + (t & 3) * 2;
+          *reinterpret_cast<float2*>(gcol + gcol_idx(row, col)) = make_float2(acc[e], acc[e + 1]);
+        }
+      }
+      named_bar_sync(1, kWorkers);
+      if (split) mma_gw_<BN, 1>(wacc, sco, sco + 16384, sgo, sgo + NKS * 8192);
+      else mma_gw_<BN, 0>(wacc, sco, sco + 16384, sgo, sgo + NKS * 8192);
+      const size_t img_off = (size_t)b * d.H * d.W * d.Cin - (size_t)(d.W + 1) * d.Cin;
+      for (int ul = 0; ul < nu; ++ul) {
+        const int tab = ntab == 2 ? ul : 0, kp = tab ? kpb : kpa, dg = tab ? dgb : dga;
+        const int cbase = sg * d.cps + (2 * m + ul - kp * d.cbs) * 64;
+        const int4* __restrict__ tp = taps + tab * 64;
+        const float* __restrict__ xc = xh + img_off + cbase + q * 4;
+        float* gc = gxh ? gxh + img_off + cbase + q * 4 : nullptr;
+        int4 tap[R];
+        Taps4 c[R];
+#pragma unroll
+        for (int j = 0; j < R; ++j) tap[j] = tp[warp * 2 * R + j * 2 + half];
+#pragma unroll
+        for (int j = 0; j < R; ++j) load_corners(xc, ucin, urs, tap[j].x, c[j]);
+#pragma unroll
+        for (int j = 0; j < R; ++j) {
+          if ((tap[j].x & 15) == 0) continue;
+          const int row = warp * 2 * R + j * 2 + half;
+          scatter_tap(c[j], tap[j], *reinterpret_cast<const float4*>(gcol + gcol_idx(row, ul * 64 + q * 4)), gc, ucin, urs,
+                      sh[j], sw[j], sm[j]);
+        }
+        if (ntab == 2 || ul == nu - 1) flush(tab, kp, dg, b, p0);
+      }
+      TapRaw raw = {0.f, 0.f, 1.f};
+      if (next && tbuild) raw = tap_loads(d, offset, mask, bn, tdg, tkp, pn + (tid & 63));
+      wgmma_wait<0>();
+      __syncwarp();
+      if (lane == 0) mbar_arrive(&empty_bar[s]);
+      named_bar_sync(1, kWorkers);
+      if (next && tbuild) taps[tid] = tap_finish(d, raw, mask != nullptr, tkp, pn + (tid & 63));
+    }
+    gw_tile_store<BN>(wacc, gw + ((size_t)sg * d.MC * 128 + (size_t)m * 128) * d.ops, d.ops);
+  } else if (warp == kWorkerWarps) {
+    if (lane == 0) {
+      const uint32_t parts = split ? 2u : 1u;
+      mbar_arrive_expect_tx(w_bar, parts * NKS * (uint32_t)kTile);
+      for (int ks = 0; ks < NKS; ++ks)
+        for (uint32_t part = 0; part < parts; ++part)
+          bulk_g2s(wres + ks * 2 * kTile + part * kTile, wt + (((size_t)sg * d.MC + m) * NKS + ks) * (2 * kTile) + part * kTile,
+                   (uint32_t)kTile, w_bar);
+      const size_t tile_bytes = parts * (size_t)kTile;
+      for (int i = 0; i < ns; ++i) {
+        const int s = i & 1;
+        const int gs = gs0 + i, b = gs / d.stages_img, st = gs - b * d.stages_img;
+        const size_t tix = ((size_t)b * d.tiles_img + (st >> 1)) * d.SG + sg, hoff = (size_t)(st & 1) * 8192;
+        uint8_t* go = stg + s * k.stage_bytes;
+        uint8_t* co = go + NKS * 16384;
+        mbar_wait(&empty_bar[s], (uint32_t)((i >> 1) & 1) ^ 1u);
+        mbar_arrive_expect_tx(&full_bar[s], parts * (uint32_t)(NKS + nu) * 8192u);
+        for (uint32_t part = 0; part < parts; ++part) {
+          for (int ks = 0; ks < NKS; ++ks)
+            bulk_g2s(go + part * (NKS * 8192) + ks * 8192, gt + (tix * NKS + ks) * (2 * kTile) + part * kTile + hoff, 8192u,
+                     &full_bar[s]);
+          for (int ul = 0; ul < nu; ++ul)
+            bulk_g2s(co + part * 16384 + ul * 8192, cols + (tix * d.U + 2 * m + ul) * tile_bytes + part * kTile + hoff, 8192u,
+                     &full_bar[s]);
+        }
+      }
+    }
+  }
+}
+
 __device__ __forceinline__ void split8(const float (&v)[8], uint4& hi, uint4& lo) {
   split2(v[0], v[1], hi.x, lo.x);
   split2(v[2], v[3], hi.y, lo.y);
@@ -1171,6 +1442,21 @@
   K2P k2;
   K3P k3;
   return make_tc(p, d) && plan_k2(d, k2) && plan_k3(d, k3);
+}
+
+static int bwd_kernels(const TC& d, int has_cols, int need_data, int need_weight, K2FP& kf) {
+  if (need_data && need_weight && has_cols && plan_k2f(d, kf)) return D2B_DCN_BWD_FUSED;
+  return (need_data ? D2B_DCN_BWD_DATA : 0) |
+         (need_weight ? (has_cols ? D2B_DCN_BWD_WEIGHT_COLS : D2B_DCN_BWD_WEIGHT) : 0);
+}
+
+int d2b_deform_conv_tc_bwd_kernels(const d2b_dcn_params* p, int has_cols, int need_data, int need_weight) {
+  TC d;
+  K2P k2;
+  K3P k3;
+  K2FP kf;
+  if (!make_tc(p, d) || !plan_k2(d, k2) || !plan_k3(d, k3)) return 0;
+  return bwd_kernels(d, has_cols, need_data, need_weight, kf);
 }
 
 size_t d2b_deform_conv_tc_fwd_workspace(const d2b_dcn_params* p, int x_nhwc) {
@@ -1313,6 +1599,8 @@
     if (grad_offset) grad_mask = grad_offset + (size_t)d.DG * 2 * d.KK * d.HoWo;
   }
   const Epi ep = {scale, nullptr, relu};
+  K2FP kf;
+  const bool fused = bwd_kernels(d, cols != nullptr, need_data, need_weight, kf) == D2B_DCN_BWD_FUSED;
   if (d.N == 0 || (!need_data && !need_weight)) {
     void* zp[3] = {grad_offset, fused_om ? nullptr : grad_mask, grad_weight};
     size_t zb[3] = {noff * 4, nm * 4, nw * 4};
@@ -1358,18 +1646,33 @@
   }
   if (need_data) {
     dcn_gout_px_tiles_kernel<<<dim3((unsigned)((size_t)d.N * d.tiles_img * d.SG * d.nks), 4), 256, 0, stream>>>(
-        grad_out, y_saved, ep, d, gt_px, gt_oc, k3.BN, k3.noct);
+        grad_out, y_saved, ep, d, gt_px, fused ? nullptr : gt_oc, k3.BN, k3.noct);
     D2B_CHECK_LAUNCH();
     {
       const long long total = (long long)d.SG * d.MC * d.nks * 128 * 8;
       dcn_wtile_bwd_kernel<<<d2b_cdiv(total, 256), 256, 0, stream>>>(weight, d, wt);
       D2B_CHECK_LAUNCH();
     }
-    const int smem_bytes = 2 * 4 * kTile + 128 * kGcolPitch * 4 + k2.tap_bytes + 1024 + 128;
-    D2B_ALLOW_BIG_SMEM(dcn_bwd_data_tc_kernel);
-    dim3 grid(d.N * d.tiles_img, d.SG, k2.msplit);
-    dcn_bwd_data_tc_kernel<<<grid, kThreads, smem_bytes, stream>>>(xh, offset, mask, gt_px, wt, d, k2, split, gxh, grad_offset,
-                                                                  mask ? grad_mask : nullptr);
+    if (fused) {
+      const int smem_bytes = k2f_smem(d, kf);
+      const uint8_t* cl = reinterpret_cast<const uint8_t*>(cols);
+      dim3 grid(d.SG * d.MC, kf.nsplit);
+#define D2B_LAUNCH_K2F(BN)                                                                                             \
+  {                                                                                                                    \
+    D2B_ALLOW_BIG_SMEM(dcn_bwd_fused_tc_kernel<BN>);                                                                   \
+    dcn_bwd_fused_tc_kernel<BN><<<grid, kThreads, smem_bytes, stream>>>(xh, offset, mask, gt_px, wt, cl, d, kf, split, gxh, \
+                                                                         grad_offset, mask ? grad_mask : nullptr, gw_part); \
+  }
+      if (d.ops == 64) D2B_LAUNCH_K2F(64)
+      else D2B_LAUNCH_K2F(128)
+#undef D2B_LAUNCH_K2F
+    } else {
+      const int smem_bytes = 2 * 4 * kTile + 128 * kGcolPitch * 4 + k2.tap_bytes + 1024 + 128;
+      D2B_ALLOW_BIG_SMEM(dcn_bwd_data_tc_kernel);
+      dim3 grid(d.N * d.tiles_img, d.SG, k2.msplit);
+      dcn_bwd_data_tc_kernel<<<grid, kThreads, smem_bytes, stream>>>(xh, offset, mask, gt_px, wt, d, k2, split, gxh,
+                                                                    grad_offset, mask ? grad_mask : nullptr);
+    }
     D2B_CHECK_LAUNCH();
     if (grad_x && !x_nhwc) {
       dim3 g2(d2b_cdiv(d.H * d.W, 64), d2b_cdiv(d.Cin, 32), d.N);
@@ -1377,7 +1680,7 @@
       D2B_CHECK_LAUNCH();
     }
   }
-  if (need_weight) {
+  if (need_weight && !fused) {
     if (!need_data) {
       const long long total = (long long)d.N * d.stages_img * d.SG * k3.noct * k3.BN * 8;
       dcn_gout_oc_tiles_kernel<<<d2b_cdiv(total, 256), 256, 0, stream>>>(grad_out, y_saved, ep, d, k3.BN, k3.noct, gt_oc);
@@ -1408,6 +1711,8 @@
 #undef D2B_LAUNCH_K3
     }
     D2B_CHECK_LAUNCH();
+  }
+  if (need_weight) {
     {
       if (d.KK <= 9) {
         dcn_gw_reduce_tile_kernel<<<dim3(d.SG * (d.cps / kRedCh), d.ops / kRedOc), 256, 0, stream>>>(gw_part, d, grad_weight);
diff --git a/detectron2_b200/csrc/deform_conv_tc.cuh b/detectron2_b200/csrc/deform_conv_tc.cuh
--- a/detectron2_b200/csrc/deform_conv_tc.cuh
+++ b/detectron2_b200/csrc/deform_conv_tc.cuh
@@ -5,6 +5,7 @@
 
 int d2b_deform_conv_tc_supported(const d2b_dcn_params* p);
 int d2b_deform_conv_tc_bwd_supported(const d2b_dcn_params* p);
+int d2b_deform_conv_tc_bwd_kernels(const d2b_dcn_params* p, int has_cols, int need_data, int need_weight);
 
 size_t d2b_deform_conv_tc_fwd_workspace(const d2b_dcn_params* p, int x_nhwc);
 size_t d2b_deform_conv_tc_cols_bytes(const d2b_dcn_params* p, int precision);
diff --git a/detectron2_b200/csrc/tc_common.cuh b/detectron2_b200/csrc/tc_common.cuh
--- a/detectron2_b200/csrc/tc_common.cuh
+++ b/detectron2_b200/csrc/tc_common.cuh
@@ -74,57 +74,57 @@
 template <int kPending>
 __device__ __forceinline__ void wgmma_wait() { asm volatile("wgmma.wait_group.sync.aligned %0;" ::"n"(kPending) : "memory"); }
 
-template <int N, int kTransA>
+template <int N, int kTransA, int kTransB = 0>
 struct Wgmma;
 
-template <int kTransA>
-struct Wgmma<8, kTransA> {
+template <int kTransA, int kTransB>
+struct Wgmma<8, kTransA, kTransB> {
   __device__ __forceinline__ static void mma(float (&d)[4], uint64_t a, uint64_t b, int accumulate) {
     asm volatile(
         "{\n\t.reg .pred p;\n\tsetp.ne.b32 p, %4, 0;\n\t"
-        "wgmma.mma_async.sync.aligned.m64n8k16.f32.bf16.bf16 {%0, %1, %2, %3}, %5, %6, p, 1, 1, %7, 0;\n\t}"
+        "wgmma.mma_async.sync.aligned.m64n8k16.f32.bf16.bf16 {%0, %1, %2, %3}, %5, %6, p, 1, 1, %7, %8;\n\t}"
         : "+f"(d[0]), "+f"(d[1]), "+f"(d[2]), "+f"(d[3])
-        : "r"(accumulate), "l"(a), "l"(b), "n"(kTransA));
+        : "r"(accumulate), "l"(a), "l"(b), "n"(kTransA), "n"(kTransB));
   }
 };
-template <int kTransA>
-struct Wgmma<16, kTransA> {
+template <int kTransA, int kTransB>
+struct Wgmma<16, kTransA, kTransB> {
   __device__ __forceinline__ static void mma(float (&d)[8], uint64_t a, uint64_t b, int accumulate) {
     asm volatile(
         "{\n\t.reg .pred p;\n\tsetp.ne.b32 p, %8, 0;\n\t"
-        "wgmma.mma_async.sync.aligned.m64n16k16.f32.bf16.bf16 {%0, %1, %2, %3, %4, %5, %6, %7}, %9, %10, p, 1, 1, %11, 0;\n\t}"
+        "wgmma.mma_async.sync.aligned.m64n16k16.f32.bf16.bf16 {%0, %1, %2, %3, %4, %5, %6, %7}, %9, %10, p, 1, 1, %11, %12;\n\t}"
         : "+f"(d[0]), "+f"(d[1]), "+f"(d[2]), "+f"(d[3]), "+f"(d[4]), "+f"(d[5]), "+f"(d[6]), "+f"(d[7])
-        : "r"(accumulate), "l"(a), "l"(b), "n"(kTransA));
+        : "r"(accumulate), "l"(a), "l"(b), "n"(kTransA), "n"(kTransB));
   }
 };
-template <int kTransA>
-struct Wgmma<32, kTransA> {
+template <int kTransA, int kTransB>
+struct Wgmma<32, kTransA, kTransB> {
   __device__ __forceinline__ static void mma(float (&d)[16], uint64_t a, uint64_t b, int accumulate) {
     asm volatile(
         "{\n\t.reg .pred p;\n\tsetp.ne.b32 p, %16, 0;\n\t"
-        "wgmma.mma_async.sync.aligned.m64n32k16.f32.bf16.bf16 {%0, %1, %2, %3, %4, %5, %6, %7, %8, %9, %10, %11, %12, %13, %14, %15}, %17, %18, p, 1, 1, %19, 0;\n\t}"
+        "wgmma.mma_async.sync.aligned.m64n32k16.f32.bf16.bf16 {%0, %1, %2, %3, %4, %5, %6, %7, %8, %9, %10, %11, %12, %13, %14, %15}, %17, %18, p, 1, 1, %19, %20;\n\t}"
         : "+f"(d[0]), "+f"(d[1]), "+f"(d[2]), "+f"(d[3]), "+f"(d[4]), "+f"(d[5]), "+f"(d[6]), "+f"(d[7]), "+f"(d[8]), "+f"(d[9]), "+f"(d[10]), "+f"(d[11]), "+f"(d[12]), "+f"(d[13]), "+f"(d[14]), "+f"(d[15])
-        : "r"(accumulate), "l"(a), "l"(b), "n"(kTransA));
+        : "r"(accumulate), "l"(a), "l"(b), "n"(kTransA), "n"(kTransB));
   }
 };
-template <int kTransA>
-struct Wgmma<64, kTransA> {
+template <int kTransA, int kTransB>
+struct Wgmma<64, kTransA, kTransB> {
   __device__ __forceinline__ static void mma(float (&d)[32], uint64_t a, uint64_t b, int accumulate) {
     asm volatile(
         "{\n\t.reg .pred p;\n\tsetp.ne.b32 p, %32, 0;\n\t"
-        "wgmma.mma_async.sync.aligned.m64n64k16.f32.bf16.bf16 {%0, %1, %2, %3, %4, %5, %6, %7, %8, %9, %10, %11, %12, %13, %14, %15, %16, %17, %18, %19, %20, %21, %22, %23, %24, %25, %26, %27, %28, %29, %30, %31}, %33, %34, p, 1, 1, %35, 0;\n\t}"
+        "wgmma.mma_async.sync.aligned.m64n64k16.f32.bf16.bf16 {%0, %1, %2, %3, %4, %5, %6, %7, %8, %9, %10, %11, %12, %13, %14, %15, %16, %17, %18, %19, %20, %21, %22, %23, %24, %25, %26, %27, %28, %29, %30, %31}, %33, %34, p, 1, 1, %35, %36;\n\t}"
         : "+f"(d[0]), "+f"(d[1]), "+f"(d[2]), "+f"(d[3]), "+f"(d[4]), "+f"(d[5]), "+f"(d[6]), "+f"(d[7]), "+f"(d[8]), "+f"(d[9]), "+f"(d[10]), "+f"(d[11]), "+f"(d[12]), "+f"(d[13]), "+f"(d[14]), "+f"(d[15]), "+f"(d[16]), "+f"(d[17]), "+f"(d[18]), "+f"(d[19]), "+f"(d[20]), "+f"(d[21]), "+f"(d[22]), "+f"(d[23]), "+f"(d[24]), "+f"(d[25]), "+f"(d[26]), "+f"(d[27]), "+f"(d[28]), "+f"(d[29]), "+f"(d[30]), "+f"(d[31])
-        : "r"(accumulate), "l"(a), "l"(b), "n"(kTransA));
+        : "r"(accumulate), "l"(a), "l"(b), "n"(kTransA), "n"(kTransB));
   }
 };
-template <int kTransA>
-struct Wgmma<128, kTransA> {
+template <int kTransA, int kTransB>
+struct Wgmma<128, kTransA, kTransB> {
   __device__ __forceinline__ static void mma(float (&d)[64], uint64_t a, uint64_t b, int accumulate) {
     asm volatile(
         "{\n\t.reg .pred p;\n\tsetp.ne.b32 p, %64, 0;\n\t"
-        "wgmma.mma_async.sync.aligned.m64n128k16.f32.bf16.bf16 {%0, %1, %2, %3, %4, %5, %6, %7, %8, %9, %10, %11, %12, %13, %14, %15, %16, %17, %18, %19, %20, %21, %22, %23, %24, %25, %26, %27, %28, %29, %30, %31, %32, %33, %34, %35, %36, %37, %38, %39, %40, %41, %42, %43, %44, %45, %46, %47, %48, %49, %50, %51, %52, %53, %54, %55, %56, %57, %58, %59, %60, %61, %62, %63}, %65, %66, p, 1, 1, %67, 0;\n\t}"
+        "wgmma.mma_async.sync.aligned.m64n128k16.f32.bf16.bf16 {%0, %1, %2, %3, %4, %5, %6, %7, %8, %9, %10, %11, %12, %13, %14, %15, %16, %17, %18, %19, %20, %21, %22, %23, %24, %25, %26, %27, %28, %29, %30, %31, %32, %33, %34, %35, %36, %37, %38, %39, %40, %41, %42, %43, %44, %45, %46, %47, %48, %49, %50, %51, %52, %53, %54, %55, %56, %57, %58, %59, %60, %61, %62, %63}, %65, %66, p, 1, 1, %67, %68;\n\t}"
         : "+f"(d[0]), "+f"(d[1]), "+f"(d[2]), "+f"(d[3]), "+f"(d[4]), "+f"(d[5]), "+f"(d[6]), "+f"(d[7]), "+f"(d[8]), "+f"(d[9]), "+f"(d[10]), "+f"(d[11]), "+f"(d[12]), "+f"(d[13]), "+f"(d[14]), "+f"(d[15]), "+f"(d[16]), "+f"(d[17]), "+f"(d[18]), "+f"(d[19]), "+f"(d[20]), "+f"(d[21]), "+f"(d[22]), "+f"(d[23]), "+f"(d[24]), "+f"(d[25]), "+f"(d[26]), "+f"(d[27]), "+f"(d[28]), "+f"(d[29]), "+f"(d[30]), "+f"(d[31]), "+f"(d[32]), "+f"(d[33]), "+f"(d[34]), "+f"(d[35]), "+f"(d[36]), "+f"(d[37]), "+f"(d[38]), "+f"(d[39]), "+f"(d[40]), "+f"(d[41]), "+f"(d[42]), "+f"(d[43]), "+f"(d[44]), "+f"(d[45]), "+f"(d[46]), "+f"(d[47]), "+f"(d[48]), "+f"(d[49]), "+f"(d[50]), "+f"(d[51]), "+f"(d[52]), "+f"(d[53]), "+f"(d[54]), "+f"(d[55]), "+f"(d[56]), "+f"(d[57]), "+f"(d[58]), "+f"(d[59]), "+f"(d[60]), "+f"(d[61]), "+f"(d[62]), "+f"(d[63])
-        : "r"(accumulate), "l"(a), "l"(b), "n"(kTransA));
+        : "r"(accumulate), "l"(a), "l"(b), "n"(kTransA), "n"(kTransB));
   }
 };
 
diff --git a/include/d2b200.h b/include/d2b200.h
--- a/include/d2b200.h
+++ b/include/d2b200.h
@@ -220,6 +220,11 @@
 
 #define D2B_DCN_X_NHWC 1
 int d2b_deform_conv_tc_shape_supported(const d2b_dcn_params* p, int backward);
+#define D2B_DCN_BWD_DATA 1
+#define D2B_DCN_BWD_WEIGHT 2
+#define D2B_DCN_BWD_WEIGHT_COLS 4
+#define D2B_DCN_BWD_FUSED 8
+int d2b_deform_conv_tc_bwd_path(const d2b_dcn_params* p, int has_cols, int need_data, int need_weight);
 size_t d2b_deform_conv_forward_workspace_bytes(const d2b_dcn_params* p, int precision, int flags);
 size_t d2b_deform_conv_cols_bytes(const d2b_dcn_params* p, int precision);
 int d2b_deform_conv_forward(const float* x, const float* offset, const float* mask,
```

After: 290.4 (median of 6 runs). 1.02x the previous value.
